# Xiaoming-Zhao/PointNav-VO

Hardware: AMD Instinct MI355X
Metric: RGB-D frame-pair VO inferences/s @341x192 (higher is better)
Workload: dtype f32

## Files before the change

include/pnvo.h:

```cpp
#ifndef PNVO_H_
#define PNVO_H_

#include <stddef.h>
#include <stdint.h>

#ifdef __cplusplus
extern "C" {
#endif

#define PNVO_OK 0
#define PNVO_ERR_ARG (-1)
#define PNVO_ERR_HIP (-2)
#define PNVO_ERR_STATE (-3)
#define PNVO_ERR_WEIGHTS (-4)
#define PNVO_ERR_INPUT (-5)

typedef struct pnvo_model_s *pnvo_handle;

typedef struct {
  int32_t width, height;
  int32_t n_rgb, n_depth, n_dd, n_tdv;
  int32_t baseplanes;
  int32_t hidden;
  int32_t out_dim;
// ... 129 lines not shown

int pnvo_policy_act(pnvo_policy_handle h, const float *depth, const float *goal, const int64_t *prev_actions,
                    const float *masks, const float *hidden_in, int B, float *hidden_out, float *features, float *logits,
                    float *value, void *stream);

int pnvo_policy_features_shape(pnvo_policy_handle h, int64_t shape[3]);
int pnvo_policy_encode(pnvo_policy_handle h, const float *depth, int B, float *features_out, void *stream);
int pnvo_policy_act_features(pnvo_policy_handle h, const float *visual_features, const float *goal, const int64_t *prev_actions,
                             const float *masks, const float *hidden_in, int B, float *hidden_out, float *features, float *logits,
                             float *value, void *stream);

int pnvo_policy_destroy(pnvo_policy_handle h);

size_t pnvo_policy_train_tail_floats(pnvo_policy_handle h);
int pnvo_policy_train_attach(pnvo_policy_handle h, float *params, float *grads, size_t n_floats, const pnvo_tensor_desc *toc,
                             int ntoc);

int pnvo_policy_train_refresh(pnvo_policy_handle h, void *stream);

int pnvo_policy_evaluate(pnvo_policy_handle h, const float *depth, const float *goal, const int64_t *prev_actions,
                         const float *masks, const float *hidden_in, int T, int N, const int64_t *actions, int train_encoder,
                         float *hidden_out, float *value, float *logp, float *entropy, void *stream);

int pnvo_policy_evaluate_features(pnvo_policy_handle h, const float *visual_features, const float *goal, const int64_t *prev_actions,
                                  const float *masks, const float *hidden_in, int T, int N, const int64_t *actions, float *hidden_out,
                                  float *value, float *logp, float *entropy, void *stream);

int pnvo_policy_ppo_loss(pnvo_policy_handle h, const float *actions_logp_old, const float *adv, const float *value_preds,
                         const float *returns, float clip, float value_coef, float entropy_coef, int use_clipped_value_loss,
                         float *out3, void *stream);

int pnvo_policy_backward(pnvo_policy_handle h, int train_encoder, void *stream);

int pnvo_policy_clip_grad_norm(pnvo_policy_handle h, float max_norm, float *norm_out, void *stream);

int pnvo_policy_train_timing(pnvo_policy_handle h, int mode);
int pnvo_policy_train_timing_read(pnvo_policy_handle h, double ms[5]);


int pnvo_rollout_insert(float *recurrent_hidden_states, int64_t *actions, int64_t *prev_actions, float *action_log_probs,
                        float *value_preds, float *rewards, float *masks, int T, int N, int64_t hidden_row, int step,
                        const float *hidden_in, const int64_t *actions_in, const float *action_log_probs_in,
                        const float *value_preds_in, const float *rewards_in, const float *masks_in, void *stream);

int pnvo_rollout_after_update(float *recurrent_hidden_states, int64_t *prev_actions, float *masks, int T, int N, int64_t hidden_row,
                              int step, void *stream);

int pnvo_rollout_compute_returns(const float *rewards, float *value_preds, const float *masks, float *returns, const float *next_value,
                                 int T, int N, int step, int use_gae, float gamma, float gamma_tau, void *stream);

int pnvo_rollout_gather(const float *recurrent_hidden_states, const int64_t *actions, const int64_t *prev_actions,
                        const float *value_preds, const float *returns, const float *masks, const float *action_log_probs,
                        const float *advantages, const int64_t *perm, int N, int L, int H, int steps, int start, int n_mb,
                        float *hidden_out, int64_t *actions_out, int64_t *prev_actions_out, float *value_preds_out, float *returns_out,
                        float *masks_out, float *action_log_probs_out, float *advantages_out, void *stream);

int pnvo_rollout_gather_frames(const float *frames, const int64_t *perm, int N, int64_t F, int steps, int start, int n_mb, float *out,
                               void *stream);

int pnvo_avgpool2(const float *depth, int N, int H, int W, float *out, void *stream);

const char *pnvo_last_error(pnvo_handle h);

const char *pnvo_last_note(pnvo_handle h);


int pnvo_set_tap(pnvo_handle h, const char *name, float *dst, size_t capacity);
int pnvo_tap_shape(pnvo_handle h, const char *name, int B, int64_t shape[4]);

typedef struct {
  char name[96];
  int64_t launches;
  double total_ms;
  double flops;
  double bytes;
} pnvo_kernel_time;
int pnvo_forward_features(pnvo_handle h, const float *rgb, const float *depth, const float *dd, const float *tdv,
                          const int64_t *actions, int B, float *hidden_out, void *stream);

int pnvo_check_inputs(pnvo_handle h);

int pnvo_layer_kernel(pnvo_handle h, const char *name, int B, char *family, size_t cap, double *executed_flops);

int pnvo_timing_mode(pnvo_handle h, int mode);
int pnvo_timing_read(pnvo_handle h, pnvo_kernel_time *entries, int cap, int *n_out);

size_t pnvo_packed_conv_floats(int cout, int cin, int kh, int kw);
int pnvo_pack_conv_weight(const float *oihw, int cout, int cin, int kh, int kw, float *out);

int pnvo_resize_area(const void *src, int src_dtype, int n, int in_h, int in_w, int channels, int64_t src_frame_stride,
                     int64_t src_row_stride, int64_t src_pix_stride, int rs_h, int rs_w, int crop_y, int crop_x, int out_h, int out_w,
                     float *dst, int dst_group, int64_t dst_group_stride, int64_t dst_member_stride, int64_t dst_row_stride,
                     int64_t dst_pix_stride, int div_rule, void *stream);

const char *pnvo_version(void);

long long pnvo_device_bytes_live(void);

#ifdef __cplusplus
}
#endif
#endif
```

pointnav-vo_amd/_lib.py:

```python
import ctypes as C
import os

import numpy as np

import torch

_HERE = os.path.dirname(os.path.abspath(__file__))
LIB_PATH = os.path.join(_HERE, "csrc", "libpnvo.so")

PNVO_OK = 0


GRAD_READY_FN = C.CFUNCTYPE(None, C.c_void_p, C.c_uint64, C.c_uint64, C.c_void_p)


class PnvoError(RuntimeError):
    pass


class pnvo_config(C.Structure):
    _fields_ = [(n, C.c_int32) for n in (
        "width", "height", "n_rgb", "n_depth", "n_dd", "n_tdv", "baseplanes", "hidden", "out_dim", "normalize",
        "act_embed", "n_acts", "flat_size", "max_batch", "backbone_depth")]

# ... 18 lines not shown
                                        C.c_void_p, C.c_void_p]),
    "pnvo_forward_grouped_raw": (C.c_int, [C.c_void_p, C.c_void_p, C.c_int, C.c_void_p, C.c_void_p, C.c_void_p, C.c_int, C.c_void_p,
                                           C.c_void_p, C.c_void_p]),
    "pnvo_grouped_supported": (C.c_int, [C.c_void_p, C.c_int]),
    "pnvo_set_precision": (C.c_int, [C.c_void_p, C.c_int]),
    "pnvo_set_option": (C.c_int, [C.c_void_p, C.c_char_p, C.c_char_p]),
    "pnvo_get_option": (C.c_int, [C.c_void_p, C.c_char_p, C.c_char_p, C.c_size_t]),
    "pnvo_forward_dual": (C.c_int, [C.c_void_p, C.c_void_p, C.c_void_p, C.c_void_p, C.c_void_p, C.c_void_p, C.c_int,
                                    C.c_void_p, C.c_void_p, C.c_void_p]),
    "pnvo_build_obs_pairs": (C.c_int, [C.c_void_p, C.c_void_p, C.c_int, C.c_int, C.c_int, C.c_int, C.POINTER(C.c_float), C.c_int,
                                       C.c_void_p, C.c_void_p, C.c_void_p, C.c_void_p, C.c_void_p, C.c_void_p, C.c_void_p]),
    "pnvo_stage_frames": (C.c_int, [C.c_void_p, C.c_int, C.c_size_t, C.c_void_p, C.c_int]),
    "pnvo_stage_frames2": (C.c_int, [C.c_void_p, C.c_size_t, C.c_void_p, C.c_void_p, C.c_size_t, C.c_void_p, C.c_int, C.c_int]),
    "pnvo_discretize_depth": (C.c_int, [C.c_void_p, C.c_int64, C.c_int64, C.c_int, C.c_void_p, C.c_int64, C.c_void_p,
                                        C.c_void_p]),
    "pnvo_topdown_workspace_bytes": (C.c_size_t, [C.c_int, C.c_int, C.c_int]),
    "pnvo_topdown_view_f64": (C.c_int, [C.c_void_p, C.c_int, C.c_int, C.c_int, C.c_int64, C.c_int64, C.c_void_p, C.c_int,
                                        C.c_void_p, C.c_int64, C.c_int64, C.c_void_p, C.c_void_p]),
    "pnvo_half_to_float": (C.c_int, [C.c_void_p, C.c_int64, C.c_void_p, C.c_void_p]),
    "pnvo_dataset_pairs": (C.c_int, [C.c_void_p] * 7 + [C.c_int] * 5 + [C.c_void_p] * 7),
    "pnvo_topdown_view_pairs": (C.c_int, [C.c_void_p, C.c_int, C.c_int, C.c_int, C.POINTER(C.c_float), C.c_int, C.c_void_p, C.c_void_p,
                                          C.c_void_p]),
    "pnvo_topdown_view": (C.c_int, [C.c_void_p, C.c_int, C.c_int, C.c_int, C.c_int64, C.c_int64,
                                    C.POINTER(C.c_float), C.c_int, C.c_void_p, C.c_int64, C.c_int64, C.c_void_p,
                                    C.c_void_p]),
    "pnvo_train_attach": (C.c_int, [C.c_void_p, C.c_void_p, C.c_void_p, C.c_size_t, C.POINTER(pnvo_tensor_desc), C.c_int]),
    "pnvo_train_refresh": (C.c_int, [C.c_void_p, C.c_void_p]),
    "pnvo_train_forward": (C.c_int, [C.c_void_p, C.c_void_p, C.c_void_p, C.c_void_p, C.c_void_p, C.c_int, C.c_void_p,
                                     C.c_void_p, C.c_void_p, C.c_void_p]),
    "pnvo_train_backward": (C.c_int, [C.c_void_p, C.c_void_p, C.c_void_p]),
    "pnvo_train_set_grad_hook": (C.c_int, [C.c_void_p, C.c_void_p, C.c_void_p]),
    "pnvo_train_grad_buckets": (C.c_int, [C.c_void_p, C.POINTER(C.c_uint64), C.POINTER(C.c_uint64), C.c_int, C.POINTER(C.c_int)]),
    "pnvo_input_moments": (C.c_int, [C.c_void_p, C.c_void_p, C.c_void_p, C.c_void_p, C.c_void_p, C.c_int, C.c_void_p,
                                     C.c_int, C.c_void_p, C.c_void_p]),
    "pnvo_rmv_merge": (C.c_int, [C.c_void_p, C.c_int, C.c_int, C.c_void_p, C.c_void_p, C.c_void_p, C.c_void_p]),
    "pnvo_train_set_actions": (C.c_int, [C.c_void_p, C.c_void_p]),
    "pnvo_mse_loss": (C.c_int, [C.c_void_p, C.c_void_p, C.c_int, C.c_int, C.c_void_p, C.c_void_p, C.c_void_p]),
    "pnvo_mse_loss_coef": (C.c_int, [C.c_void_p, C.c_void_p, C.c_void_p, C.c_int, C.c_void_p, C.c_void_p, C.c_void_p]),
    "pnvo_geo_inverse_loss": (C.c_int, [C.c_void_p, C.c_void_p, C.c_int, C.c_int, C.c_float, C.c_void_p, C.c_void_p,
                                        C.c_void_p]),
    "pnvo_train_set_dropout": (C.c_int, [C.c_void_p, C.c_float, C.c_uint64]),
    "pnvo_train_dropout_mask": (C.c_int, [C.c_void_p, C.c_int, C.c_void_p, C.c_void_p]),
    "pnvo_adam_step": (C.c_int, [C.c_void_p, C.c_void_p, C.c_void_p, C.c_void_p, C.c_size_t, C.c_float, C.c_float,
                                 C.c_float, C.c_float, C.c_int, C.c_void_p]),
    "pnvo_destroy": (C.c_int, [C.c_void_p]),
    "pnvo_ring_assemble": (C.c_int, [C.c_void_p, C.c_void_p, C.c_void_p, C.c_void_p, C.c_void_p, C.c_void_p, C.c_void_p, C.c_int, C.c_int,
                                     C.c_int, C.c_void_p, C.c_void_p, C.c_void_p, C.c_void_p]),
    "pnvo_last_error": (C.c_char_p, [C.c_void_p]),
    "pnvo_last_note": (C.c_char_p, [C.c_void_p]),
    "pnvo_set_tap": (C.c_int, [C.c_void_p, C.c_char_p, C.c_void_p, C.c_size_t]),
    "pnvo_tap_shape": (C.c_int, [C.c_void_p, C.c_char_p, C.c_int, C.POINTER(C.c_int64)]),
    "pnvo_check_inputs": (C.c_int, [C.c_void_p]),
    "pnvo_forward_features": (C.c_int, [C.c_void_p, C.c_void_p, C.c_void_p, C.c_void_p, C.c_void_p, C.c_void_p, C.c_int,
                                        C.c_void_p, C.c_void_p]),
    "pnvo_policy_create": (C.c_int, [C.c_void_p, C.c_int, C.POINTER(C.c_void_p)]),
    "pnvo_policy_load_weights": (C.c_int, [C.c_void_p, C.c_void_p, C.c_size_t, C.c_void_p, C.c_int]),
    "pnvo_policy_act": (C.c_int, [C.c_void_p, C.c_void_p, C.c_void_p, C.c_void_p, C.c_void_p, C.c_void_p, C.c_int,
                                  C.c_void_p, C.c_void_p, C.c_void_p, C.c_void_p, C.c_void_p]),
    "pnvo_policy_features_shape": (C.c_int, [C.c_void_p, C.POINTER(C.c_int64)]),
    "pnvo_policy_encode": (C.c_int, [C.c_void_p, C.c_void_p, C.c_int, C.c_void_p, C.c_void_p]),
    "pnvo_policy_act_features": (C.c_int, [C.c_void_p, C.c_void_p, C.c_void_p, C.c_void_p, C.c_void_p, C.c_void_p, C.c_int,
                                           C.c_void_p, C.c_void_p, C.c_void_p, C.c_void_p, C.c_void_p]),
    "pnvo_policy_evaluate_features": (C.c_int, [C.c_void_p, C.c_void_p, C.c_void_p, C.c_void_p, C.c_void_p, C.c_void_p, C.c_int, C.c_int,
                                                C.c_void_p, C.c_void_p, C.c_void_p, C.c_void_p, C.c_void_p, C.c_void_p]),
    "pnvo_policy_destroy": (C.c_int, [C.c_void_p]),
    "pnvo_policy_train_tail_floats": (C.c_size_t, [C.c_void_p]),
    "pnvo_policy_train_attach": (C.c_int, [C.c_void_p, C.c_void_p, C.c_void_p, C.c_size_t, C.POINTER(pnvo_tensor_desc), C.c_int]),
    "pnvo_policy_train_refresh": (C.c_int, [C.c_void_p, C.c_void_p]),
    "pnvo_policy_evaluate": (C.c_int, [C.c_void_p, C.c_void_p, C.c_void_p, C.c_void_p, C.c_void_p, C.c_void_p, C.c_int, C.c_int,
                                       C.c_void_p, C.c_int, C.c_void_p, C.c_void_p, C.c_void_p, C.c_void_p, C.c_void_p]),
    "pnvo_policy_ppo_loss": (C.c_int, [C.c_void_p, C.c_void_p, C.c_void_p, C.c_void_p, C.c_void_p, C.c_float, C.c_float, C.c_float,
                                       C.c_int, C.c_void_p, C.c_void_p]),
    "pnvo_policy_backward": (C.c_int, [C.c_void_p, C.c_int, C.c_void_p]),
    "pnvo_policy_clip_grad_norm": (C.c_int, [C.c_void_p, C.c_float, C.c_void_p, C.c_void_p]),
    "pnvo_policy_train_timing": (C.c_int, [C.c_void_p, C.c_int]),
    "pnvo_policy_train_timing_read": (C.c_int, [C.c_void_p, C.POINTER(C.c_double)]),
    "pnvo_rollout_insert": (C.c_int, [C.c_void_p] * 7 + [C.c_int, C.c_int, C.c_int64, C.c_int] + [C.c_void_p] * 7),
    "pnvo_rollout_after_update": (C.c_int, [C.c_void_p] * 3 + [C.c_int, C.c_int, C.c_int64, C.c_int, C.c_void_p]),
    "pnvo_rollout_compute_returns": (C.c_int, [C.c_void_p] * 5 + [C.c_int] * 4 + [C.c_float, C.c_float, C.c_void_p]),
    "pnvo_rollout_gather": (C.c_int, [C.c_void_p] * 9 + [C.c_int] * 6 + [C.c_void_p] * 9),
    "pnvo_rollout_gather_frames": (C.c_int, [C.c_void_p, C.c_void_p, C.c_int, C.c_int64] + [C.c_int] * 3 + [C.c_void_p, C.c_void_p]),
    "pnvo_avgpool2": (C.c_int, [C.c_void_p, C.c_int, C.c_int, C.c_int, C.c_void_p, C.c_void_p]),
    "pnvo_layer_kernel": (C.c_int, [C.c_void_p, C.c_char_p, C.c_int, C.c_char_p, C.c_size_t, C.POINTER(C.c_double)]),
    "pnvo_timing_mode": (C.c_int, [C.c_void_p, C.c_int]),
    "pnvo_timing_read": (C.c_int, [C.c_void_p, C.POINTER(pnvo_kernel_time), C.c_int, C.POINTER(C.c_int)]),
    "pnvo_packed_conv_floats": (C.c_size_t, [C.c_int, C.c_int, C.c_int, C.c_int]),
    "pnvo_pack_conv_weight": (C.c_int, [C.c_void_p, C.c_int, C.c_int, C.c_int, C.c_int, C.c_void_p]),
    "pnvo_resize_area": (C.c_int, [C.c_void_p, C.c_int, C.c_int, C.c_int, C.c_int, C.c_int, C.c_int64, C.c_int64, C.c_int64,
                                   C.c_int, C.c_int, C.c_int, C.c_int, C.c_int, C.c_int, C.c_void_p, C.c_int, C.c_int64, C.c_int64,
                                   C.c_int64, C.c_int64, C.c_int, C.c_void_p]),
    "pnvo_version": (C.c_char_p, []),
    "pnvo_device_bytes_live": (C.c_longlong, []),
}


def _load():
    if not os.path.exists(LIB_PATH):
        raise PnvoError(
            f"{LIB_PATH} is missing: the HIP extension has not been built.  Run "
            "`python -c 'import __graft_entry__ as g; g.build()'` (or `make -C pointnav-vo_amd/csrc`).  "
            "There is no CPU fallback.")
    lib = C.CDLL(LIB_PATH)
    for name, (res, args) in _SIGNATURES.items():
        fn = getattr(lib, name)
        fn.restype = res
        fn.argtypes = args
    return lib


lib = _load()


def check(rc, handle=None):
    if rc != PNVO_OK:
        msg = lib.pnvo_last_error(handle)
        raise PnvoError(f"libpnvo error {rc}: {msg.decode() if msg else '?'}")


def make_toc(entries):
    toc = (pnvo_tensor_desc * len(entries))()
    for i, (name, offset, shape) in enumerate(entries):
        toc[i].name = name.encode()
        toc[i].offset = int(offset)
        toc[i].ndim = len(shape)
        for k, s in enumerate(shape):
            toc[i].shape[k] = int(s)
    return toc


def pack_tensors(named_tensors):
    blob = np.ascontiguousarray(np.concatenate(
        [t.detach().to("cpu", torch.float32).reshape(-1).numpy() for _, t in named_tensors]), dtype=np.float32)
    entries, off = [], 0
    for name, t in named_tensors:
        entries.append((name, off, tuple(t.shape)))
        off += t.numel()
    return blob, make_toc(entries)


def version():
    return lib.pnvo_version().decode()
```

pointnav-vo_amd/csrc/conv_rows.hip:

```cpp
#include <cstdio>
#include <cstdlib>

#include "pnvo_internal.h"

namespace pnvo {

typedef float f32x16 __attribute__((ext_vector_type(16)));
typedef float f32x4 __attribute__((ext_vector_type(4)));
typedef float f32x2 __attribute__((ext_vector_type(2)));
typedef _Float16 f16x8 __attribute__((ext_vector_type(8)));
typedef _Float16 f16x2 __attribute__((ext_vector_type(2)));
typedef unsigned u32x4 __attribute__((ext_vector_type(4)));
typedef unsigned u32x2 __attribute__((ext_vector_type(2)));

#ifndef PNVO_ROWS_ABL
#define PNVO_ROWS_ABL 0
#endif
#if PNVO_ROWS_ABL
#define RS_DBG(p) ((p).rs_dbg)
#else
#define RS_DBG(p) 0
#endif

namespace {
constexpr int RS_THREADS = 512;
constexpr int RS_HG = 128;
constexpr int RS_RING = 512;
constexpr int RS_TAIL = 48;
constexpr int RS_PITCH = 144;
constexpr int RS_RAW = (RS_RING + RS_TAIL) * RS_PITCH;
constexpr int RS_OTAB = RS_RAW + 4 * 16384;
constexpr int RS_MTAB = RS_OTAB + 4 * RS_HG * 4;
constexpr int RS_SS = RS_MTAB + 4 * RS_HG * 4;
constexpr int RS_RED = RS_SS + 64 * 4;
constexpr int RS_DOF = RS_RED + 8 * 32 * 2 * 4;
constexpr int RS_LDS = RS_DOF + 512 * 16;

__device__ __forceinline__ void rs_barrier() { asm volatile("s_waitcnt lgkmcnt(0)\n\ts_barrier" ::: "memory"); }

__device__ __forceinline__ unsigned rs_pack2h(float a, float b) {
  const f16x2 r = __builtin_convertvector(f32x2{a, b}, f16x2);
  return __builtin_bit_cast(unsigned, r);
}
}

template <int MODE>
__global__ __launch_bounds__(RS_THREADS) __attribute__((amdgpu_waves_per_eu(2, 2))) void conv_rows32_kernel(const ConvX3Args p) {
  extern __shared__ __attribute__((aligned(16))) unsigned char lds[];
  const int tid = (int)threadIdx.x;
  const int lane = tid & 63;
  const int wave = __builtin_amdgcn_readfirstlane(tid >> 6);
  const int set = wave >> 2, sw = wave & 3, stid = tid & 255;
  const int H = p.H, W = p.W, P = W + 2;
  const int nbands = p.rs_bands, brows = p.rs_rows;
  const int nitems = p.B * nbands;
  const int dR = (2 * RS_HG) / P, dC = 2 * RS_HG - dR * P;

  u32x4 bres[18][2];
#pragma unroll
  for (int st = 0; st < 18; ++st)
#pragma unroll
    for (int pc = 0; pc < 2; ++pc)
      bres[st][pc] = *reinterpret_cast<const u32x4 *>(reinterpret_cast<const char *>(p.wpk) + (size_t)st * 2048u + pc * 1024 + lane * 16);
  const float os = p.oscale_ptr != nullptr ? *p.oscale_ptr : p.oscale;

  const int q = stid & 7, jb = stid >> 3;
  int q_ = q, jb_ = jb, lane_ = lane;
  unsigned *otab = reinterpret_cast<unsigned *>(lds + RS_OTAB) + set * 2 * RS_HG;
  float *mtab = reinterpret_cast<float *>(lds + RS_MTAB) + set * 2 * RS_HG;
  float *red = reinterpret_cast<float *>(lds + RS_RED);
  float *sstab = reinterpret_cast<float *>(lds + RS_SS);
  const unsigned rawbase = (unsigned)(RS_RAW + set * 32768 + sw * 4096);

  const unsigned tbytes = (unsigned)p.B * (unsigned)(H * W * 128);
  const __amdgpu_buffer_rsrc_t rx = __builtin_amdgcn_make_buffer_rsrc((void *)p.x, 0, tbytes, 0x00020000);
  const __amdgpu_buffer_rsrc_t ry = __builtin_amdgcn_make_buffer_rsrc((void *)p.y, 0, tbytes, 0x00020000);
  const __amdgpu_buffer_rsrc_t rres = __builtin_amdgcn_make_buffer_rsrc((void *)(MODE == 2 ? p.res : p.x), 0, tbytes, 0x00020000);
  const __amdgpu_buffer_rsrc_t rxo = __builtin_amdgcn_make_buffer_rsrc((void *)(MODE >= 2 ? p.xout : p.y), 0, tbytes, 0x00020000);

  for (int item = (int)blockIdx.x; item < nitems; item += (int)gridDim.x) {
    const int n = item / nbands, band = item - n * nbands;
    const int rb = band * brows, re = min(H, rb + brows);
    const int O0 = (rb + 1) * P;
    const int nout = (re - rb) * P;
    const int NH = (nout + RS_HG - 1) / RS_HG;
    const int nbase = n * H * W * 128;
    if (MODE >= 1 && tid < 64) sstab[tid] = tid < 32 ? p.in_scale[(size_t)n * 32 + tid] : p.in_shift[(size_t)n * 32 + tid - 32];
    const int r_lo = max(rb - 1, 0), r_hi = min(re, H - 1);
    int iR, iC, iD;
    {
      const int f = O0 - 2 * RS_HG + RS_HG * (1 + set) + jb + 256 * P;
      iR = f / P - 256;
      iC = f - (iR + 256) * P;
      iD = (((iR - 1) * W + iC - 1) * 32 + 4 * q) * 4 + nbase;
    }
    int oR = 0, oC = 0, oD = 0;
    if (stid < RS_HG) {
      const int f = O0 + RS_HG * set + stid;
      oR = f / P;
      oC = f - oR * P;
      oD = ((oR - 1) * W + oC - 1) * 128 + nbase;
    }

    unsigned vok = 0, vokn = 0;
    u32x4 *const dofp = reinterpret_cast<u32x4 *>(lds + RS_DOF) + tid;
    auto issue = [&](int slot) {
      vokn = 0;
      unsigned off[4];
      u32x4 dn = {0, 0, 0, 0};
#pragma unroll
      for (int k = 0; k < 4; ++k) {
        const int r32 = (32 * k) / P, c32 = 32 * k - r32 * P;
        const int cw = iC + c32 >= P ? 1 : 0;
        const int R = iR + r32 + cw, Cc = iC + c32 - cw * P;
        const bool ok = (unsigned)(R - 1 - r_lo) <= (unsigned)(r_hi - r_lo) && (unsigned)(Cc - 1) < (unsigned)W;
        const unsigned dense = (unsigned)(iD + (32 * k - 2 * (r32 + cw)) * 128), absent = ok ? 0u : 0x80000000u;
        off[k] = ok ? dense - 1024u * k : 0x80000000u;
        vokn |= ok ? (1u << k) : 0u;
        if (MODE >= 2) {
          dn[k] = dense | absent;
          vokn |= (ok && (unsigned)(R - 1 - rb) < (unsigned)(re - rb)) ? (16u << k) : 0u;
        }
      }
      if (MODE >= 2) *dofp = dn;
      if (!(RS_DBG(p) & 1)) {
        const unsigned m0v = rawbase + (unsigned)slot * 16384u;
        asm volatile(
            "s_mov_b32 m0, %5\n\ts_nop 0\n\t"
            "buffer_load_dwordx4 %0, %4, 0 offen lds\n\t"
            "buffer_load_dwordx4 %1, %4, 0 offen offset:1024 lds\n\t"
// ... 120 lines not shown
          a[1] = *reinterpret_cast<const u32x4 *>(lds + arow[0] + 64);
#pragma unroll
          for (int st = 0; st < 18; ++st) {
            if (st + 1 < 18) {
              const int nt = (st + 1) >> 1, nk = (st + 1) & 1;
              an[0] = *reinterpret_cast<const u32x4 *>(lds + arow[nt / 3] + (nt % 3) * RS_PITCH + nk * 32);
              an[1] = *reinterpret_cast<const u32x4 *>(lds + arow[nt / 3] + (nt % 3) * RS_PITCH + nk * 32 + 64);
            }
            f32x16 &c = (TWO_ACC && (st & 1)) ? acc1 : acc;
            c = __builtin_amdgcn_mfma_f32_32x32x16_f16(__builtin_bit_cast(f16x8, a[1]), __builtin_bit_cast(f16x8, bres[st][0]), c, 0, 0, 0);
            c = __builtin_amdgcn_mfma_f32_32x32x16_f16(__builtin_bit_cast(f16x8, a[0]), __builtin_bit_cast(f16x8, bres[st][1]), c, 0, 0, 0);
            c = __builtin_amdgcn_mfma_f32_32x32x16_f16(__builtin_bit_cast(f16x8, a[0]), __builtin_bit_cast(f16x8, bres[st][0]), c, 0, 0, 0);
            a[0] = an[0];
            a[1] = an[1];
          }
          if (TWO_ACC) {
#pragma unroll
            for (int r = 0; r < 16; ++r) acc[r] += acc1[r];
          }
          if (EPI_IN_COMPUTE) epilogue(h);
        }
      } else {
        asm volatile("s_waitcnt vmcnt(0)" ::: "memory");
#if PNVO_ROWS_ABL
        pt1 = __builtin_readcyclecounter();
        pc_wait += pt1 - pt0;
#endif
        asm volatile("" : "+v"(q_), "+v"(jb_), "+v"(lane_));
        vok = vokn;
        if (MODE >= 2) dof = *dofp;
        if (MODE == 2) load_skip();
        if (h + 6 <= NH + 2) issue((duty + 1) & 1);
        if (!EPI_IN_COMPUTE && h >= 1) epilogue(h - 1);
        if (h + 4 <= NH + 2 && !(RS_DBG(p) & 8)) convert_store(h + 4, duty & 1);

        if (h + 1 >= 0 && h + 1 < NH) tables(h + 1);
        ++duty;
      }
#if PNVO_ROWS_ABL
      const unsigned long long pt2 = __builtin_readcyclecounter();
      if ((h & 1) == set) pc_compute += pt2 - pt0; else pc_stage += pt2 - pt1;
#endif
      rs_barrier();
#if PNVO_ROWS_ABL
      pc_bar += __builtin_readcyclecounter() - pt2;
#endif
    }
#if PNVO_ROWS_ABL
    if (p.prof != nullptr && item == 7 && lane == 0) {
      unsigned long long *d = p.prof + wave * 8;
      d[0] = pc_compute; d[1] = pc_stage; d[2] = pc_bar; d[3] = pc_wait; d[4] = (unsigned long long)(NH + 4);
    }
#endif

    if (p.stats != nullptr) {
      t1 += __shfl_xor(t1, 32);
      t2 += __shfl_xor(t2, 32);
      if (lane < 32) *reinterpret_cast<f32x2 *>(red + (wave * 32 + lane) * 2) = f32x2{t1, t2};
      __syncthreads();
      if (wave == 0 && lane < 32) {
        float s1 = 0.f, s2 = 0.f;
#pragma unroll
        for (int w = 0; w < 8; ++w) {
          const f32x2 o = *reinterpret_cast<const f32x2 *>(red + (w * 32 + lane) * 2);
          s1 += o[0];
          s2 += o[1];
        }
        float *dst = p.stats + (((size_t)n * p.slots + band) * 32 + lane) * 2;
        dst[0] = s1;
        dst[1] = s2;
        if (p.gn_scale != nullptr) {
          const int c = lane;
          const bool first = p.gn_mu != nullptr && c % p.gn_cpg == 0;
          const long gi = (long)n * (32 / p.gn_cpg) + c / p.gn_cpg;
          gn_finalize_lane(s1, s2, p.gn_cpg, p.gn_P, p.gn_eps, p.gn_gamma[c], p.gn_beta[c], p.gn_scale + (size_t)n * 32 + c,
                           p.gn_shift + (size_t)n * 32 + c, first ? p.gn_mu + gi : nullptr, first ? p.gn_rstd + gi : nullptr);
        }
      }
    }
    __syncthreads();
  }
}

bool conv_rows32_plan(ConvX3Args &a, int ks, int stride, int mode, int num_cus) {
  if (ks != 3 || stride != 1 || a.np != 2 || a.CIN != 32 || a.COUTP != 32 || a.in_absmax != nullptr) return false;
  if (mode < 0 || mode > 3 || (mode == 2 && a.res_scale != nullptr)) return false;
  if (a.Ho != a.H || a.Wo != a.W || a.W + 3 > RS_HG || a.W < 8 || a.H < 8 || (long)a.B * a.H * a.W * 128 >= (1L << 31)) return false;
  int bands = 1;
  while ((long)a.B * bands < num_cus && bands < 4 && a.H / (bands * 2) >= 12) bands *= 2;
  if ((long)a.B * bands < num_cus) return false;
  if (const char *e = std::getenv("PNVO_ROWS_DBG")) a.rs_dbg = std::atoi(e);
  a.rs_rows = (a.H + bands - 1) / bands;
  a.rs_bands = (a.H + a.rs_rows - 1) / a.rs_rows;
  a.slots = a.rs_bands;
  return true;
}

hipError_t launch_conv_rows32(const ConvX3Args &a, int mode, int num_cus, hipStream_t s) {
  static std::mutex attr_mu;
  static unsigned long long attr_seen = 0;
  if (pnvo_first_launch_on_device(attr_mu, attr_seen)) {
    hipError_t e = hipFuncSetAttribute(reinterpret_cast<const void *>(conv_rows32_kernel<0>), hipFuncAttributeMaxDynamicSharedMemorySize, RS_LDS);
    if (e == hipSuccess)
      e = hipFuncSetAttribute(reinterpret_cast<const void *>(conv_rows32_kernel<1>), hipFuncAttributeMaxDynamicSharedMemorySize, RS_LDS);
    if (e == hipSuccess)
      e = hipFuncSetAttribute(reinterpret_cast<const void *>(conv_rows32_kernel<2>), hipFuncAttributeMaxDynamicSharedMemorySize, RS_LDS);
    if (e == hipSuccess)
      e = hipFuncSetAttribute(reinterpret_cast<const void *>(conv_rows32_kernel<3>), hipFuncAttributeMaxDynamicSharedMemorySize, RS_LDS);
    if (e != hipSuccess) return e;
  }
  const long items = (long)a.B * a.rs_bands;
  const unsigned gx = (unsigned)(items < num_cus ? items : num_cus);
  ConvX3Args q = a;
#if PNVO_ROWS_ABL
  static unsigned long long *prof = nullptr;
  if (std::getenv("PNVO_ROWS_PROF") != nullptr) {
    if (!prof && hipMalloc((void **)&prof, 8 * 8 * 8) != hipSuccess) return hipErrorOutOfMemory;
    (void)hipMemsetAsync(prof, 0, 8 * 8 * 8, s);
    q.prof = prof;
  }
#endif
  if (mode == 0)
    hipLaunchKernelGGL((conv_rows32_kernel<0>), dim3(gx), dim3(RS_THREADS), RS_LDS, s, q);
  else if (mode == 1)
    hipLaunchKernelGGL((conv_rows32_kernel<1>), dim3(gx), dim3(RS_THREADS), RS_LDS, s, q);
  else if (mode == 2)
    hipLaunchKernelGGL((conv_rows32_kernel<2>), dim3(gx), dim3(RS_THREADS), RS_LDS, s, q);
  else if (mode == 3)
    hipLaunchKernelGGL((conv_rows32_kernel<3>), dim3(gx), dim3(RS_THREADS), RS_LDS, s, q);
  else
    return hipErrorInvalidValue;
#if PNVO_ROWS_ABL
  if (q.prof != nullptr) {
    unsigned long long h[64];
    (void)hipStreamSynchronize(s);
    (void)hipMemcpy(h, prof, sizeof(h), hipMemcpyDeviceToHost);
    for (int w = 0; w < 8; w += 3)
      std::fprintf(stderr, "[pnvo] conv_rows32 wave %d: per half-step (cycles): compute role %.0f  stage role %.0f (+ wait for its loads/stores %.0f)  barrier %.0f  (%llu half-steps)\n",
                   w, 2.0 * h[8 * w] / h[8 * w + 4], 2.0 * h[8 * w + 1] / h[8 * w + 4], 2.0 * h[8 * w + 3] / h[8 * w + 4], (double)h[8 * w + 2] / h[8 * w + 4], h[8 * w + 4]);
  }
#endif
  return hipGetLastError();
}

}
```

pointnav-vo_amd/csrc/conv_x3.hip:

```cpp
#include <cmath>
#include <cstdio>
#include <cstdlib>
#include <cstring>

#include "pnvo_internal.h"

namespace pnvo {

typedef float f32x16 __attribute__((ext_vector_type(16)));
typedef float f32x4 __attribute__((ext_vector_type(4)));
typedef float f32x2 __attribute__((ext_vector_type(2)));
typedef __bf16 bf16x8 __attribute__((ext_vector_type(8)));
typedef __bf16 bf16x2 __attribute__((ext_vector_type(2)));
typedef _Float16 f16x8 __attribute__((ext_vector_type(8)));
typedef _Float16 f16x2 __attribute__((ext_vector_type(2)));
typedef unsigned u32x4 __attribute__((ext_vector_type(4)));

namespace {
__device__ __forceinline__ unsigned pack2(float a, float b) {
  const bf16x2 r = __builtin_convertvector(f32x2{a, b}, bf16x2);
  return __builtin_bit_cast(unsigned, r);
}
__device__ __forceinline__ unsigned pack2h(float a, float b) {
  const f16x2 r = __builtin_convertvector(f32x2{a, b}, f16x2);
  return __builtin_bit_cast(unsigned, r);
}
__device__ __forceinline__ float lo_f(unsigned u) { return __builtin_bit_cast(float, u << 16); }
__device__ __forceinline__ float hi_f(unsigned u) { return __builtin_bit_cast(float, u & 0xffff0000u); }
}

constexpr int x3_wpe(int mw, int nw, int np, bool dsf = false) {
  return dsf ? (mw * nw >= 6 ? 1 : (mw * nw >= 2 ? 2 : 3)) : ((np == 2 && mw * nw <= 2) ? 3 : 2);
}

template <int KS, int STRIDE, int MODE, int MW, int NW, int NP, bool DSF = false, bool W8 = false, bool KSW = false>
__global__ __launch_bounds__(W8 ? 512 : 256) __attribute__((amdgpu_waves_per_eu(W8 ? 2 : x3_wpe(MW, NW, NP, DSF), W8 ? 2 : x3_wpe(MW, NW, NP, DSF)))) void conv_x3_kernel(const ConvX3Args p) {
  constexpr int NTH = W8 ? 512 : 256, NWV = NTH / 64;
  constexpr int EMW = KSW ? 1 : MW;
  static_assert(!KSW || (NW == 1 && NP == 2 && KS == 3 && !DSF && !W8), "K split over the waves: float16-piece 3x3 convs, one N-tile");
  static_assert(!DSF || (KS == 3 && STRIDE == 2 && NP == 2 && (MODE == 0 || MODE == 2)), "the downsample rides on a float16-piece 3x3 stride-2 conv");
  extern __shared__ __attribute__((aligned(16))) unsigned char lds[];
  constexpr int PSTEP = KS == 1 ? STRIDE : 1;
  constexpr int CS = KS == 1 ? 1 : STRIDE;
  constexpr int PAD = KS / 2;
  const int lane = threadIdx.x & 63;
  const int wave = __builtin_amdgcn_readfirstlane(threadIdx.x >> 6);

  const int ntiles = p.B * p.tiles_r * p.tiles_c;
  const int chunk = (ntiles + 7) >> 3;
  int bid = (int)(blockIdx.x & 7) * chunk + (int)(blockIdx.x >> 3);
  if (bid >= ntiles) return;
  const int tci = bid % p.tiles_c;
  bid /= p.tiles_c;
  const int tri = bid % p.tiles_r;
  const int n = bid / p.tiles_r;
  const int r0 = tri * p.TR, c0 = tci * p.TC;
  const int hi0 = r0 * STRIDE - PAD, wi0 = c0 * STRIDE - PAD;
  const int mdl = (p.grp_end0 > 0 && n >= p.grp_end0) + (p.grp_end1 > 0 && n >= p.grp_end1);
  const unsigned short *g_wpk = mdl == 0 ? p.wpk : p.wpk_g[mdl - 1];
  const unsigned short *g_ds_wpk = mdl == 0 ? p.ds_wpk : p.ds_wpk_g[mdl - 1];
  const float g_oscale = mdl == 0 ? p.oscale : p.oscale_g[mdl - 1], g_ds_oscale = mdl == 0 ? p.ds_oscale : p.ds_oscale_g[mdl - 1];
  const float *g_gamma = mdl == 0 ? p.gn_gamma : p.gn_gamma_g[mdl - 1], *g_beta = mdl == 0 ? p.gn_beta : p.gn_beta_g[mdl - 1];
  const float *g_ds_gamma = mdl == 0 ? p.ds_gamma : p.ds_gamma_g[mdl - 1], *g_ds_beta = mdl == 0 ? p.ds_beta : p.ds_beta_g[mdl - 1];
  const int PR = p.PR, PC = p.PC, CK = p.CK;
  const int pitch = CK * 2 + 16;
  const int plane = PR * PC * pitch;
  const int npix = p.TR * p.TC;
  const int tab_off = KSW ? max(NP * plane, 4 * MW * 4096) : NP * plane;
  unsigned *qtab = reinterpret_cast<unsigned *>(lds + tab_off);
  unsigned *otab = qtab + p.MT * 32;
  for (int e = (int)threadIdx.x; e < p.MT * 32; e += NTH) {
    const int q = min(e, npix - 1);
    const int tr = q / p.TC, tc = q - tr * p.TC;
    qtab[e] = (unsigned)(((tr * CS) * PC + tc * CS) * pitch);
    const bool ok = e < npix && r0 + tr < p.Ho && c0 + tc < p.Wo;
    otab[e] = (unsigned)((tr * p.Wo + tc) * p.COUTP) | (ok ? 0u : 0x80000000u);
  }

  const int wn = p.wn;
  const int wave_m = wave / wn;
  const int wave_n = (wave & (wn - 1)) + (int)blockIdx.y * wn;
  const int ntt = p.COUTP >> 5, kct = p.CIN >> 4;

  f32x16 acc[MW][NW];
#pragma unroll
  for (int i = 0; i < MW; ++i)
#pragma unroll
    for (int j = 0; j < NW; ++j)
#pragma unroll
      for (int r = 0; r < 16; ++r) acc[i][j][r] = 0.f;
  f32x16 accd[DSF ? MW : 1][DSF ? NW : 1];
  if (DSF) {
#pragma unroll
    for (int i = 0; i < MW; ++i)
#pragma unroll
      for (int j = 0; j < NW; ++j)
#pragma unroll
        for (int r = 0; r < 16; ++r) accd[DSF ? i : 0][DSF ? j : 0][r] = 0.f;
  }

  float in_mul = 1.f, in_div = 1.f;
  const bool in_scaled = NP == 2 && p.in_absmax != nullptr;
  if (in_scaled) {
    unsigned mb = p.in_absmax[(threadIdx.x & 63) * 16];
#pragma unroll
    for (int d = 32; d >= 1; d >>= 1) mb = max(mb, (unsigned)__shfl_xor((int)mb, d));
    const int e = mb != 0u ? (int)((mb >> 23) & 0xffu) - 126 : 14;
    in_mul = __builtin_bit_cast(float, (unsigned)(14 - e + 127) << 23);
    in_div = __builtin_bit_cast(float, (unsigned)(e - 14 + 127) << 23);
  }
  const int G = CK >> 3;
  const int cg = threadIdx.x & (G - 1), pl = threadIdx.x / G, PS = NTH / G;
  const int dr = PS / PC, dc = PS - dr * PC;
  const int nppix = PR * PC;

  unsigned long long c_stage = 0, c_mm = 0, t_0 = __builtin_readcyclecounter(), r_0 = wall_clock64();
  for (int ck0 = 0; ck0 < p.CIN; ck0 += CK) {
    unsigned long long t_a = __builtin_readcyclecounter();
    if (ck0 > 0) __syncthreads();
// ... 416 lines not shown
      u32x4 ent[4];
#pragma unroll
      for (int g4 = 0; g4 < 4; ++g4) ent[g4] = *reinterpret_cast<const u32x4 *>(otab + mt * 32 + 8 * g4 + 4 * rr16);
      unsigned flags = 0;
#pragma unroll
      for (int g4 = 0; g4 < 4; ++g4) flags |= ent[g4][0] | ent[g4][1] | ent[g4][2] | ent[g4][3];
      const bool whole = !__any((int)(flags >> 31));
#pragma unroll
      for (int j = 0; j < NW; ++j) {
        const int nt = wave_n * NW + j;
        if (nt >= ntt) continue;
        const int co = nt * 32 + (lane & 31);
        float s1 = 0.f, s2 = 0.f;
        if (whole) {
#pragma unroll
          for (int r = 0; r < 16; ++r) {
            const float v = ac[i][j][r];
            (yout + ybase + co)[ent[r >> 2][r & 3]] = v;
            s1 += v;
            s2 = __builtin_fmaf(v, v, s2);
          }
        } else {
#pragma unroll
          for (int r = 0; r < 16; ++r) {
            const unsigned e = ent[r >> 2][r & 3];
            const bool ok = (int)e >= 0;
            const float v = ok ? ac[i][j][r] : 0.f;
            if (ok) (yout + ybase + co)[e] = v;
            s1 += v;
            s2 = __builtin_fmaf(v, v, s2);
          }
        }
        t1[j] += s1 + __shfl_xor(s1, 32);
        t2[j] += s2 + __shfl_xor(s2, 32);
      }
    }
    if (stats != nullptr) {
      const int rows = NWV / wn;
      float *red = reinterpret_cast<float *>(lds);
      if (rows > 1) {
        __syncthreads();
        if (lane < 32)
#pragma unroll
          for (int j = 0; j < NW; ++j) *reinterpret_cast<f32x2 *>(red + ((wave * NW + j) * 32 + lane) * 2) = f32x2{t1[j], t2[j]};
        __syncthreads();
      }
      if (wave_m == 0 && lane < 32) {
#pragma unroll
        for (int j = 0; j < NW; ++j) {
          const int nt = wave_n * NW + j;
          if (nt >= ntt) continue;
          float s1 = t1[j], s2 = t2[j];
          for (int w = 1; w < rows; ++w) {
            const f32x2 o = *reinterpret_cast<const f32x2 *>(red + (((w * wn + (wave & (wn - 1))) * NW + j) * 32 + lane) * 2);
            s1 += o[0];
            s2 += o[1];
          }
          float *dst = stats + (((long)n * p.slots + tri * p.tiles_c + tci) * p.COUTP + nt * 32 + lane) * 2;
          dst[0] = s1;
          dst[1] = s2;
          if (gscale != nullptr) {
            const int c = nt * 32 + lane;
            const bool first = gmu != nullptr && c % p.gn_cpg == 0;
            const long gi = (long)n * (p.COUTP / p.gn_cpg) + c / p.gn_cpg;
            gn_finalize_lane(s1, s2, p.gn_cpg, p.gn_P, p.gn_eps, gamma[c], beta[c], gscale + (long)n * p.COUTP + c,
                             gshift + (long)n * p.COUTP + c, first ? gmu + gi : nullptr, first ? grstd + gi : nullptr);
          }
        }
      }
    }
    (void)again;
  };
  emit(acc, p.y, p.stats, p.oscale_ptr, g_oscale, g_gamma, g_beta, p.gn_scale, p.gn_shift, p.gn_mu, p.gn_rstd, false);
  if constexpr (DSF) emit(accd, p.ds_y, p.ds_stats, p.ds_oscale_ptr, g_ds_oscale, g_ds_gamma, g_ds_beta, p.ds_scale, p.ds_shift, p.ds_mu, p.ds_rstd, true);
  if (p.prof && lane == 0 && blockIdx.x == 13 && blockIdx.y == 0) {
    const unsigned long long t_f = __builtin_readcyclecounter();
    unsigned long long *d = p.prof + wave * 8;
    d[0] = c_stage;
    d[1] = c_mm;
    d[2] = t_f - t_e;
    d[3] = t_f - t_0;
    d[4] = wall_clock64() - r_0;
  }
}


template <int MODE, int MW, int NW, bool BRES>
__global__ __launch_bounds__(256) __attribute__((amdgpu_waves_per_eu(BRES ? 2 : 3, BRES ? 2 : 3))) void conv_x3p_kernel(const ConvX3Args p) {
  static_assert(MODE == 0 || MODE == 1 || MODE == 3, "the block-tail stager has no registers for a second patch");
  static_assert(!BRES || NW == 1, "resident weights: one N-tile");
  extern __shared__ __attribute__((aligned(16))) unsigned char lds[];
  constexpr int KS = 3, PAD = 1, NP = 2;
  const int lane = threadIdx.x & 63;
  const int wave = __builtin_amdgcn_readfirstlane(threadIdx.x >> 6);
  const int ntiles = p.B * p.tiles_r * p.tiles_c;
  const int chunk = (ntiles + 7) >> 3;
  const int PR = p.PR, PC = p.PC, CK = p.CK;
  const int pitch = CK * 2 + 16;
  const int plane = PR * PC * pitch;
  const int npix = p.TR * p.TC;
  unsigned *qtab = reinterpret_cast<unsigned *>(lds + NP * plane);
  unsigned *otab = qtab + p.MT * 32;
  const int wn = p.wn;
  const int wave_m = wave / wn;
  const int wave_n = (wave & (wn - 1)) + (int)blockIdx.y * wn;
  const int ntt = p.COUTP >> 5;
  float in_mul = 1.f, in_div = 1.f;
  const bool in_scaled = p.in_absmax != nullptr;
  if (in_scaled) {
    unsigned mb = p.in_absmax[(threadIdx.x & 63) * 16];
#pragma unroll
    for (int d = 32; d >= 1; d >>= 1) mb = max(mb, (unsigned)__shfl_xor((int)mb, d));
    const int e = mb != 0u ? (int)((mb >> 23) & 0xffu) - 126 : 14;
    in_mul = __builtin_bit_cast(float, (unsigned)(14 - e + 127) << 23);
    in_div = __builtin_bit_cast(float, (unsigned)(e - 14 + 127) << 23);
  }
  const int G = CK >> 3;
  const int cg = threadIdx.x & (G - 1), pl = threadIdx.x / G, PS = 256 / G;
  const int nppix = PR * PC;
  constexpr int NPX = 6;
  int ppr[NPX], ppc[NPX];
  unsigned poff[NPX];
  bool pok[NPX];
#pragma unroll
  for (int k = 0; k < NPX; ++k) {
    const int pix = pl + k * PS;
    pok[k] = pix < nppix;
    const int q = pok[k] ? pix : 0;
    ppr[k] = q / PC;
    ppc[k] = q - ppr[k] * PC;
    poff[k] = (unsigned)((ppr[k] * PC + ppc[k]) * pitch + 16 * cg);
  }
  if ((int)threadIdx.x < p.MT * 32) {
    const int q = min((int)threadIdx.x, npix - 1);
    const int tr = q / p.TC, tc = q - tr * p.TC;
    qtab[threadIdx.x] = (unsigned)((tr * PC + tc) * pitch);
  }
  struct Tile {
    int n, tri, tci, r0, c0, hi0, wi0;
    bool valid;
  };
  auto decode = [&](int vb) {
    Tile t;
    int bid = (vb & 7) * chunk + (vb >> 3);
    t.valid = vb < 8 * chunk && bid < ntiles;
    if (!t.valid) bid = 0;
    t.tci = bid % p.tiles_c;
    bid /= p.tiles_c;
    t.tri = bid % p.tiles_r;
    t.n = bid / p.tiles_r;
    t.r0 = t.tri * p.TR;
    t.c0 = t.tci * p.TC;
    t.hi0 = t.r0 - PAD;
    t.wi0 = t.c0 - PAD;
    return t;
  };
  f32x4 v[NPX][2], sc0, sc1, sh0, sh1;
  bool inb[NPX];
  auto fetch = [&](const Tile &t) {
    const long img = ((long)t.n * p.H * p.W) * p.CIN + 8 * cg;
    if (MODE >= 1) {
      const float *ps = p.in_scale + (long)t.n * p.CIN + 8 * cg;
      const float *pt = p.in_shift + (long)t.n * p.CIN + 8 * cg;
      sc0 = *reinterpret_cast<const f32x4 *>(ps);
      sc1 = *reinterpret_cast<const f32x4 *>(ps + 4);
      sh0 = *reinterpret_cast<const f32x4 *>(pt);
// ... 223 lines not shown
          }
        } else {
#pragma unroll
          for (int r = 0; r < 16; ++r) {
            const unsigned e = ent[r >> 2][r & 3];
            const bool ok = (int)e >= 0;
            const float x = ok ? acc[i][j][r] : 0.f;
            if (ok) (p.y + ybase + co)[e] = x;
            s1 += x;
            s2 = __builtin_fmaf(x, x, s2);
          }
        }
        t1[j] += s1 + __shfl_xor(s1, 32);
        t2[j] += s2 + __shfl_xor(s2, 32);
      }
    }
    if (p.stats != nullptr) {
      const int rows = 4 / wn;
      float *red = reinterpret_cast<float *>(lds);
      if (rows > 1) {
        __syncthreads();
        if (lane < 32)
#pragma unroll
          for (int j = 0; j < NW; ++j) *reinterpret_cast<f32x2 *>(red + ((wave * NW + j) * 32 + lane) * 2) = f32x2{t1[j], t2[j]};
        __syncthreads();
      }
      if (wave_m == 0 && lane < 32) {
#pragma unroll
        for (int j = 0; j < NW; ++j) {
          const int nt = wave_n * NW + j;
          if (nt >= ntt) continue;
          float s1 = t1[j], s2 = t2[j];
          for (int w = 1; w < rows; ++w) {
            const f32x2 o = *reinterpret_cast<const f32x2 *>(red + (((w * wn + (wave & (wn - 1))) * NW + j) * 32 + lane) * 2);
            s1 += o[0];
            s2 += o[1];
          }
          float *dst = p.stats + (((long)cur.n * p.slots + cur.tri * p.tiles_c + cur.tci) * p.COUTP + nt * 32 + lane) * 2;
          dst[0] = s1;
          dst[1] = s2;
        }
      }
    }
    if (!nxt.valid) break;
    if (BRES) fetch(nxt);
    __syncthreads();
    cur = nxt;
  }
}

namespace {
template <int KS, int STRIDE, int NP>
hipError_t launch_ks(const ConvX3Args &a, int mode, int mw, int nw, dim3 grid, size_t ldsb, hipStream_t s) {
#define PNVO_X3(MODE_, MW_, NW_)                                                                          \
  if (mode == MODE_ && mw == MW_ && nw == NW_) {                                                          \
    hipLaunchKernelGGL((conv_x3_kernel<KS, STRIDE, MODE_, MW_, NW_, NP>), grid, dim3(256), ldsb, s, a);   \
    return hipGetLastError();                                                                             \
  }
  if constexpr (KS == 3 && STRIDE == 2 && NP == 2) {
    if (a.ds_wpk != nullptr) {
#define PNVO_X3D(MODE_, MW_, NW_)                                                                               \
  if (mode == MODE_ && mw == MW_ && nw == NW_) {                                                                \
    hipLaunchKernelGGL((conv_x3_kernel<KS, STRIDE, MODE_, MW_, NW_, NP, true>), grid, dim3(256), ldsb, s, a);   \
    return hipGetLastError();                                                                                   \
  }
      if (a.w8) {
#define PNVO_X3DW(MODE_)                                                                                                  \
  if (mode == MODE_ && mw == 3 && nw == 1) {                                                                             \
    hipLaunchKernelGGL((conv_x3_kernel<KS, STRIDE, MODE_, 3, 1, NP, true, true>), grid, dim3(512), ldsb, s, a);          \
    return hipGetLastError();                                                                                            \
  }
        PNVO_X3DW(0) PNVO_X3DW(2)
#undef PNVO_X3DW
        return hipErrorInvalidValue;
      }
      PNVO_X3D(0, 1, 1) PNVO_X3D(2, 1, 1) PNVO_X3D(0, 2, 1) PNVO_X3D(2, 2, 1) PNVO_X3D(0, 2, 2) PNVO_X3D(2, 2, 2) PNVO_X3D(0, 3, 2) PNVO_X3D(2, 3, 2)
#undef PNVO_X3D
      return hipErrorInvalidValue;
    }
  }
  PNVO_X3(0, 1, 1) PNVO_X3(1, 1, 1) PNVO_X3(0, 2, 1) PNVO_X3(1, 2, 1) PNVO_X3(0, 2, 2) PNVO_X3(1, 2, 2) PNVO_X3(0, 3, 2) PNVO_X3(1, 3, 2)
  PNVO_X3(2, 1, 1) PNVO_X3(2, 2, 1) PNVO_X3(2, 2, 2) PNVO_X3(2, 3, 2) PNVO_X3(3, 1, 1) PNVO_X3(3, 2, 1) PNVO_X3(3, 2, 2) PNVO_X3(3, 3, 2)

  if (KS == 3 && STRIDE == 1 && NP == 2) {
    PNVO_X3(0, 5, 1) PNVO_X3(1, 5, 1) PNVO_X3(2, 5, 1) PNVO_X3(3, 5, 1)
    if constexpr (KS == 3 && STRIDE == 1 && NP == 2) if (a.ksw) {
#define PNVO_X3K(MODE_, MW_)                                                                                             \
  if (mode == MODE_ && mw == MW_ && nw == 1) {                                                                          \
    hipLaunchKernelGGL((conv_x3_kernel<KS, STRIDE, MODE_, MW_, 1, NP, false, false, true>), grid, dim3(256), ldsb, s, a); \
    return hipGetLastError();                                                                                           \
  }
      PNVO_X3K(0, 3) PNVO_X3K(1, 3) PNVO_X3K(2, 3) PNVO_X3K(0, 4) PNVO_X3K(1, 4) PNVO_X3K(2, 4)
#undef PNVO_X3K
      return hipErrorInvalidValue;
    }
  }
  if constexpr (KS == 3 && NP == 2) if (a.w8) {
#define PNVO_X3W(MODE_)                                                                                                  \
  if (mode == MODE_ && mw == 3 && nw == 1) {                                                                            \
  hipLaunchKernelGGL((conv_x3_kernel<KS, STRIDE, MODE_, 3, 1, NP, false, true>), grid, dim3(512), ldsb, s, a);        \
  return hipGetLastError();                                                                                           \
  }
    PNVO_X3W(0) PNVO_X3W(1) PNVO_X3W(2) PNVO_X3W(3)
#undef PNVO_X3W
    return hipErrorInvalidValue;
  }
#undef PNVO_X3
  return hipErrorInvalidValue;
}
}

namespace {
bool conv_x3_plan_impl(ConvX3Args &a, int ks, int stride, int *mw, int *nw, size_t *lds_bytes, bool fine);
long plan_wgs(const ConvX3Args &a, int nw) {
  const int ntt = a.COUTP / 32;
  return (long)a.B * a.tiles_r * a.tiles_c * ((ntt + a.wn * nw - 1) / (a.wn * nw));
}
}

bool conv_x3_plan(ConvX3Args &a, int ks, int stride, int *mw, int *nw, size_t *lds_bytes) {
  ConvX3Args reg = a;
  int rmw = 0, rnw = 0;
  size_t rlds = 0;
  const int force0 = a.force;
  reg.force = 1;
  const bool reg_ok = conv_x3_plan_impl(reg, ks, stride, &rmw, &rnw, &rlds, false);
  const long reg_wgs = reg_ok ? plan_wgs(reg, rnw) : 0;
  const int ntt = a.COUTP / 32;
  if (a.fine && a.np == 2 && ntt >= 2 && (!reg_ok || reg_wgs < 224)) {
    ConvX3Args f = a;
    int fmw = 0, fnw = 0;
    size_t flds = 0;
    f.force = 1;
    if (conv_x3_plan_impl(f, ks, stride, &fmw, &fnw, &flds, true)) {
      const long fw = plan_wgs(f, fnw);
      if (fw > reg_wgs && (fw >= 48 || force0)) {
        f.force = force0;
        a = f;
        *mw = fmw;
        *nw = fnw;
        *lds_bytes = flds;
        return true;
      }
    }
  }
  return conv_x3_plan_impl(a, ks, stride, mw, nw, lds_bytes, false);
}

namespace {
bool conv_x3_plan_impl(ConvX3Args &a, int ks, int stride, int *mw, int *nw, size_t *lds_bytes, bool fine) {
  if (a.CIN % 32 || a.COUTP % 32 || a.COUTP > 1024 || a.CIN > 1024) return false;
  if (!((ks == 3 && (stride == 1 || stride == 2)) || (ks == 1 && stride == 2))) return false;
  a.w8 = 0;
  a.ksw = 0;
  const int ntt = a.COUTP / 32;
  int TR, TC;
  if (stride == 2 && ks == 3) {
    TC = a.Wo >= 32 ? 16 : a.Wo;
    const int pc = 2 * TC + 1;
    TR = (324 / pc - 1) / 2;
    if (TR < 1) return false;
    if (TR > a.Ho) TR = a.Ho;
    while (TR > 1 && TR * TC > (ntt == 2 ? 64 : (ntt == 4 ? 128 : 96))) --TR;
  } else if (ntt == 1 && stride == 1 && ks == 3 && a.CIN > 32 && a.np == 2 && a.Wo < 32 && a.Ho * a.Wo <= 128) {
    TC = a.Wo;
    TR = a.Ho;
  } else if (ntt == 1) {
    if (stride != 1 || ks != 3 || a.CIN != 32) return false;
    TC = a.Wo >= 16 ? 16 : a.Wo;
    TR = 256 / TC;
    while (TR > 1 && (TR + 2) * (TC + 2) > 324) --TR;
    if (TR > a.Ho) TR = a.Ho;
    if (TR * TC <= 96) return false;
  } else if (a.strip && !fine && a.np == 2 && stride == 1 && ks == 3 && ntt == 4 && a.Wo >= 16 && a.Ho >= 8) {
    const int ncol = (a.Wo + 21) / 22;
    TC = (a.Wo + ncol - 1) / ncol;
    TR = 288 / TC;
    if (TR > a.Ho) TR = a.Ho;
    const int nrow = (a.Ho + TR - 1) / TR;
    TR = (a.Ho + nrow - 1) / nrow;
  } else if (a.Wo >= 32) {
    TR = 8;
    TC = 16;
  } else {
    TC = a.Wo;
    int target = ntt == 4 ? 192 : (ntt >= 8 ? 96 : 128);
    if (fine && a.ksw_ok && ks == 3 && stride == 1 && a.np == 2 && a.CIN >= 128) target = 96;
    TR = target / TC;
    if (TR < 1) TR = 1;
    if (TR > a.Ho) TR = a.Ho;
  }
  a.TR = TR;
  a.TC = TC;
  a.tiles_r = (a.Ho + TR - 1) / TR;
  a.tiles_c = (a.Wo + TC - 1) / TC;
  a.MT = (TR * TC + 31) / 32;
  const int cs = ks == 1 ? 1 : stride;
  a.PR = (TR - 1) * cs + ks;
  a.PC = (TC - 1) * cs + ks;
  const bool strip = a.strip && !fine && a.np == 2 && stride == 1 && ks == 3 && ntt == 4 && a.Wo >= 16 && a.Ho >= 8 && a.MT > 6;
  if (fine) {
    if (a.MT > 8) return false;
    a.wn = 1;
    *mw = (a.MT + 3) / 4;
    *nw = 1;
    if (a.ksw_ok && (a.MT == 3 || a.MT == 4) && ks == 3 && stride == 1 && a.np == 2 && a.CIN >= 128) {
      a.ksw = 1;
      *mw = a.MT;
    }
  } else if (strip) {
    a.wn = 2;
    *mw = (a.MT + 1) / 2;
    *nw = 1;
    if (*mw > 5) return false;
    if (*mw < 5) *mw = 5;
  } else if (ntt == 1) {
    a.wn = 1;
    *mw = a.CIN > 32 ? 1 : 2;
    *nw = 1;
    if (a.ksw_ok && a.CIN >= 128 && (a.MT == 3 || a.MT == 4) && ks == 3 && stride == 1 && a.np == 2) {
      a.ksw = 1;
      *mw = a.MT;
    }
  } else if (ntt == 2) {
    a.wn = 2;
    *mw = a.MT > 2 ? 2 : 1;
    *nw = 1;
  } else if (ntt == 4) {
    a.wn = 2;
    *mw = a.MT > 4 ? 3 : 2;
    *nw = 2;
  } else {
    a.wn = 4;
    *mw = a.MT > 2 ? 3 : 2;
    *nw = 2;
    const long ntiles = (long)a.B * a.tiles_r * a.tiles_c;
    if (ntiles < 200 && a.MT <= 4) {
      a.wn = 2;
      *mw = 2;
    }
    if (a.w8_ok && !fine && ntiles >= 200 && a.MT == 3 && ntt == 8 && a.np == 2 && ks == 3) {
      a.w8 = 1;
      a.wn = 8;
      *mw = 3;
      *nw = 1;
    }
  }
  if (!a.ksw && ((a.w8 ? 8 : 4) / a.wn) * *mw < a.MT) return false;
  const size_t np = a.np == 2 ? 2 : 3;
  int ck = 32;
  while (ck < 256 && a.CIN % (2 * ck) == 0) ck *= 2;
  const size_t cap = (size_t)72 * 1024;
  while (ck > 32 && np * a.PR * a.PC * (ck * 2 + 16) > cap) ck /= 2;
  if (np * a.PR * a.PC * (ck * 2 + 16) > cap + 4096) return false;
  if (a.CIN % ck) return false;
  a.CK = ck;
  {
    const bool force = a.force != 0;
    const long wgs = (long)a.B * a.tiles_r * a.tiles_c * ((ntt + a.wn * *nw - 1) / (a.wn * *nw));
    if (wgs < (a.np == 2 ? 112 : 192) && !force) return false;
  }
  a.slots = a.tiles_r * a.tiles_c;
  *lds_bytes = np * a.PR * a.PC * (ck * 2 + 16) + (size_t)a.MT * 32 * 4 * 2;
  if (a.ksw) *lds_bytes = std::max(np * a.PR * a.PC * (ck * 2 + 16), (size_t)4 * a.MT * 4096) + (size_t)a.MT * 32 * 4 * 2;
  return true;
}
}

bool conv_x3_persistent(const ConvX3Args &a, int ks, int stride, int mode, int mw, int nw) {
  const long ntiles = (long)a.B * a.tiles_r * a.tiles_c;
  const int ntt = a.COUTP / 32, pwgs = a.persist_wgs;
  const bool bres = ntt == 1 && a.CIN == 32 && nw == 1 && (mode == 0 || mode == 1);
  return a.np == 2 && ks == 3 && stride == 1 && bres && mw * nw <= 2 && a.CK == a.CIN && pwgs >= 8 &&
         (long)a.PR * a.PC * (a.CK / 8) <= 6 * 256 && ntiles >= 2L * pwgs;
}

hipError_t launch_conv_x3(const ConvX3Args &a0, int ks, int stride, int mode, int mw, int nw, size_t lds_bytes, hipStream_t s) {
  ConvX3Args a = a0;
  static unsigned long long *prof = nullptr;
  static const bool want = std::getenv("PNVO_X3_PROF") != nullptr;
  if (want && !prof) {
    (void)hipMalloc((void **)&prof, 512);
    (void)hipMemset(prof, 0, 512);
  }
  a.prof = prof;
  struct Dump {
    const ConvX3Args &a; int mw, nw; hipStream_t s; unsigned long long *prof;
    ~Dump() {
      static int calls = 0;
      if (!prof || ++calls > 40) return;
      unsigned long long h[64];
      (void)hipStreamSynchronize(s);
      (void)hipMemcpy(h, prof, 512, hipMemcpyDeviceToHost);
      std::fprintf(stderr, "[pnvo] conv_x3 B %d %dx%d cin %d cout %d tile %dx%d MT %d CK %d (%d,%d) wn %d: wave0 stage %llu mfma %llu epi %llu total %llu "
                           "(100MHz ticks %llu) | wave3 stage %llu mfma %llu epi %llu total %llu\n", a.B, a.Ho, a.Wo, a.CIN, a.COUTP, a.TR, a.TC,
                   a.MT, a.CK, mw, nw, a.wn, h[0], h[1], h[2], h[3], h[4], h[24], h[25], h[26], h[27]);
    }
  } dump{a, mw, nw, s, prof};
  const long ntiles = (long)a.B * a.tiles_r * a.tiles_c;
  const int ntt = a.COUTP / 32, per_wg = a.wn * nw;
  dim3 grid((unsigned)(((ntiles + 7) / 8) * 8), (unsigned)((ntt + per_wg - 1) / per_wg), 1u);
  const int pwgs = a.persist_wgs;
  if (conv_x3_persistent(a, ks, stride, mode, mw, nw)) {
    const bool bres = true;
    dim3 pg((unsigned)(pwgs & ~7), grid.y, 1u);
    if (bres) pg.x = (unsigned)(((pwgs / 3) * 2) & ~7);
#define PNVO_X3P(MODE_, MW_, NW_)                                                                        \
  if (mode == MODE_ && mw == MW_ && nw == NW_) {                                                         \
    hipLaunchKernelGGL((conv_x3p_kernel<MODE_, MW_, NW_, true>), pg, dim3(256), lds_bytes, s, a);       \
    return hipGetLastError();                                                                            \
  }
    PNVO_X3P(0, 1, 1) PNVO_X3P(1, 1, 1) PNVO_X3P(0, 2, 1) PNVO_X3P(1, 2, 1)
#undef PNVO_X3P
  }
  if (a.np == 2) {
    if (ks == 3 && stride == 1) return launch_ks<3, 1, 2>(a, mode, mw, nw, grid, lds_bytes, s);
    if (ks == 3 && stride == 2) return launch_ks<3, 2, 2>(a, mode, mw, nw, grid, lds_bytes, s);
    if (ks == 1 && stride == 2) return launch_ks<1, 2, 2>(a, mode, mw, nw, grid, lds_bytes, s);
    return hipErrorInvalidValue;
  }
  if (ks == 3 && stride == 1) return launch_ks<3, 1, 3>(a, mode, mw, nw, grid, lds_bytes, s);
  if (ks == 3 && stride == 2) return launch_ks<3, 2, 3>(a, mode, mw, nw, grid, lds_bytes, s);
  if (ks == 1 && stride == 2) return launch_ks<1, 2, 3>(a, mode, mw, nw, grid, lds_bytes, s);
  return hipErrorInvalidValue;
}

void pack_conv_x3_weight(const float *oihw, int cout, int cin, int cinp, int coutp, int kh_, int kw_, unsigned short *out) {
  const int T = kh_ * kw_, kct = cinp / 16, ntt = coutp / 32;
  auto bf = [](float f) {
    unsigned u;
    std::memcpy(&u, &f, 4);
    if ((u & 0x7f800000u) == 0x7f800000u) return (unsigned short)(u >> 16);
    u += 0x7fffu + ((u >> 16) & 1u);
    return (unsigned short)(u >> 16);
  };
  auto tof = [](unsigned short h) {
    const unsigned u = (unsigned)h << 16;
    float f;
    std::memcpy(&f, &u, 4);
    return f;
  };
  for (int tap = 0; tap < T; ++tap)
    for (int kc = 0; kc < kct; ++kc)
      for (int nt = 0; nt < ntt; ++nt)
        for (int ln = 0; ln < 64; ++ln)
          for (int j = 0; j < 8; ++j) {
            const int co = nt * 32 + (ln & 31), ci = 16 * kc + 8 * (ln >> 5) + j;
            float v = 0.f;
            if (co < cout && ci < cin) v = oihw[((size_t)co * cin + ci) * T + tap];
            const unsigned short h = bf(v);
            const float r1 = v - tof(h);
            const unsigned short m = bf(r1);
            const unsigned short l = bf(r1 - tof(m));
            const size_t base = ((((size_t)tap * kct + kc) * ntt + nt) * 3) * 64 * 8 + (size_t)ln * 8 + j;
            out[base] = h;
            out[base + 64 * 8] = m;
            out[base + 2 * 64 * 8] = l;
          }
}

static unsigned short f32_to_f16_rne(float f) {
  const _Float16 h = (_Float16)f;
  unsigned short u;
  std::memcpy(&u, &h, 2);
  return u;
}
static float f16_to_f32(unsigned short u) {
  _Float16 h;
  std::memcpy(&h, &u, 2);
  return (float)h;
}
float pack_conv_x2_weight(const float *oihw, int cout, int cin, int cinp, int coutp, int kh_, int kw_, unsigned short *out) {
  const int T = kh_ * kw_, kct = cinp / 16, ntt = coutp / 32;
  float mx = 0.f;
  for (size_t k = 0; k < (size_t)cout * cin * T; ++k) mx = std::fmax(mx, std::fabs(oihw[k]));
  int e = 0;
  if (mx > 0.f) std::frexp(mx, &e);
  const float scale = std::ldexp(1.0f, 12 - e), inv = std::ldexp(1.0f, e - 12);
  for (int tap = 0; tap < T; ++tap)
    for (int kc = 0; kc < kct; ++kc)
      for (int nt = 0; nt < ntt; ++nt)
        for (int ln = 0; ln < 64; ++ln)
          for (int j = 0; j < 8; ++j) {
            const int co = nt * 32 + (ln & 31), ci = 16 * kc + 8 * (ln >> 5) + j;
            float v = 0.f;
            if (co < cout && ci < cin) v = oihw[((size_t)co * cin + ci) * T + tap] * scale;
            const unsigned short h = f32_to_f16_rne(v);
            const unsigned short m = f32_to_f16_rne(v - f16_to_f32(h));
            const size_t base = ((((size_t)tap * kct + kc) * ntt + nt) * 2) * 64 * 8 + (size_t)ln * 8 + j;
            out[base] = h;
            out[base + 64 * 8] = m;
          }
  return inv;
}

__global__ __launch_bounds__(256) void conv_x3_repack_kernel(const float *w, int cout, int cin, int cinp, int coutp, int T,
                                                           int transposed, unsigned short *out, long total) {
  const long e = (long)blockIdx.x * 256 + threadIdx.x;
  if (e >= total) return;
  const int j = (int)(e & 7), ln = (int)((e >> 3) & 63);
  long r = e >> 9;
  const int ntt = coutp / 32, kct = cinp / 16;
  const int nt = (int)(r % ntt);
  r /= ntt;
  const int kc = (int)(r % kct), tap = (int)(r / kct);
  const int co = nt * 32 + (ln & 31), ci = 16 * kc + 8 * (ln >> 5) + j;
  const float v = (co < cout && ci < cin) ? (transposed ? w[((long)ci * cout + co) * T + (T - 1 - tap)] : w[((long)co * cin + ci) * T + tap])
// ... 86 lines not shown
```

pointnav-vo_amd/csrc/pnvo_api.hip:

```cpp
#include <hip/hip_runtime.h>

#include <cmath>
#include <cstdio>
#include <cstdlib>
#include <cstring>
#include <functional>
#include <atomic>
#include <condition_variable>
#include <map>
#include <mutex>
#include <string>
#include <thread>
#include <vector>

#include "pnvo_model.h"

using namespace pnvo;

thread_local std::string g_err;

int pnvo_fail(pnvo_handle h, int code, const std::string &msg) {
  if (h) h->err = msg;
  g_err = msg;
  return code;
}

long long pnvo_device_bytes_live(void) { return g_device_bytes_live.load(); }

namespace {

inline int fail(pnvo_handle h, int code, const std::string &msg) { return pnvo_fail(h, code, msg); }


Layer make_layer(const std::string &name, const std::string &gn, int cin, int cout, int k, int stride, int pad,
                 int hin, int win, int groups) {
  Layer l;
  l.name = name;
  l.gn = gn;
  l.cin = cin;
  l.cinp = rup(cin, 8);
  l.cout = cout;
  l.coutp = rup(cout, 32);
  l.k = l.kw = k;
  l.stride = stride;
  l.pad = pad;
  l.hin = hin;
  l.win = win;
  l.hout = (hin + 2 * pad - k) / stride + 1;
  l.wout = (win + 2 * pad - k) / stride + 1;
  l.groups = groups;
  return l;
}

void build_plan(pnvo_model_s *m) {
  const pnvo_config &c = m->cfg;
  m->C = c.n_rgb + c.n_depth + c.n_dd + c.n_tdv;
  m->CP = rup(m->C, 8);
  m->CPL = rup(m->C, 16);
  m->Hs = halve(c.height);
  m->Ws = halve(c.width);
  m->Hp = halve(m->Hs);
  m->Wp = halve(m->Ws);
  {
    const int n[4] = {c.n_rgb, c.n_depth, c.n_dd, c.n_tdv};
    int prev_off[4], half = 0;
    for (int t = 0; t < 4; ++t) {
      prev_off[t] = half;
      half += n[t] / 2;
    }
    m->stem_ref_of_new.clear();
    m->stem_tensor_of_new.clear();
    m->stem_ch_of_new.clear();
    for (int t = 0; t < 4; ++t)
      for (int ch = 0; ch < n[t]; ++ch) {
        const int hn = n[t] / 2;
        m->stem_ref_of_new.push_back(ch < hn ? prev_off[t] + ch : half + prev_off[t] + (ch - hn));
        m->stem_tensor_of_new.push_back(t);
        m->stem_ch_of_new.push_back(ch);
      }
    while ((int)m->stem_ref_of_new.size() < m->CP) {
      m->stem_ref_of_new.push_back(-1);
      m->stem_tensor_of_new.push_back(-1);
      m->stem_ch_of_new.push_back(0);
    }
  }
  const int g = c.baseplanes / 2;
  const std::string bb = "visual_encoder.backbone.";
  m->convs.clear();
  m->convs.push_back(make_layer(bb + "conv1.0", bb + "conv1.1", m->C, c.baseplanes, 7, 2, 3, c.height, c.width, g));
  int h = m->Hp, w = m->Wp, cin = c.baseplanes;
  const bool bott = c.backbone_depth == 50 || c.backbone_depth == 101;
  const int nblk[4] = {bott ? 3 : 2, bott ? 4 : 2, bott ? (c.backbone_depth == 101 ? 23 : 6) : 2, bott ? 3 : 2};
  m->bottleneck = bott;
  m->blocks.clear();
  auto push = [&](Layer l) {
    l.block = (int)m->blocks.size();
    m->convs.push_back(std::move(l));
// ... 74 lines not shown
    s += "])";
    *rc = fail(h, PNVO_ERR_WEIGHTS, s);
    return nullptr;
  }
  return t.blob + d->offset;
}

}

void pnvo_pack_conv_weight_cinp(const float *oihw, int cout, int cin, int cinp, int kh, int kw, std::vector<float> &out) {
  const int coutp = rup(cout, 32), J = cinp / 8, T = kh * kw, ntg_n = coutp / 32;
  out.assign((size_t)coutp * cinp * T, 0.f);
  for (int ntg = 0; ntg < ntg_n; ++ntg)
    for (int tap = 0; tap < T; ++tap)
      for (int j = 0; j < J; ++j)
        for (int hh = 0; hh < 2; ++hh)
          for (int n = 0; n < 32; ++n)
            for (int t = 0; t < 4; ++t) {
              const int co = ntg * 32 + n, ci = 8 * j + 4 * hh + t;
              if (co < cout && ci < cin)
                out[((((size_t)ntg * T + tap) * J + j) * 64 + hh * 32 + n) * 4 + t] =
                    oihw[((size_t)co * cin + ci) * T + tap];
            }
}

namespace {
inline void pack_conv_weight_cinp(const float *oihw, int cout, int cin, int cinp, int kh, int kw, std::vector<float> &out) {
  pnvo_pack_conv_weight_cinp(oihw, cout, cin, cinp, kh, kw, out);
}

int load_conv(pnvo_handle h, const Toc &t, Layer &l, bool has_gn) {
  int rc = PNVO_OK;
  const float *w = find_tensor(h, t, l.name + ".weight", {l.cout, l.cin, l.k, l.kw}, &rc);
  if (!w) return rc;
  std::vector<float> pk;
  pack_conv_weight_cinp(w, l.cout, l.cin, l.cinp, l.k, l.kw, pk);
  HIPCHK(h, l.wpk.upload(pk.data(), pk.size()));
  l.host_w.assign(w, w + (size_t)l.cout * l.cin * l.k * l.kw);
  if (has_gn) {
    const float *g = find_tensor(h, t, l.gn + ".weight", {l.cout}, &rc);
    if (!g) return rc;
    const float *b = find_tensor(h, t, l.gn + ".bias", {l.cout}, &rc);
    if (!b) return rc;
    HIPCHK(h, l.gamma.upload(g, l.cout));
    HIPCHK(h, l.beta.upload(b, l.cout));
  }
  return PNVO_OK;
}

int reset_contract_flag(pnvo_handle h) {
  if (!h->dd_flag) HIPCHK(h, h->dd_flag.alloc_host(1, hipHostMallocMapped | hipHostMallocCoherent));
  if (!h->dd_flag_dev) HIPCHK(h, h->dd_flag_dev.alloc(1));
  *(volatile int *)h->dd_flag = 0;
  HIPCHK(h, hipMemset(h->dd_flag_dev, 0, sizeof(int)));
  return PNVO_OK;
}

void free_workspace(pnvo_model_s *m) {
  pnvo_drop_graphs(m);
  for (DevBuf<float> *b : {&m->xin, &m->stem_raw, &m->out_ws, &m->bufY[0], &m->bufY[1], &m->rawA, &m->rawB, &m->rawD, &m->rawC, &m->comp_raw,
                           &m->hid, &m->stats, &m->stats_ds, &m->tapbuf})
    b->reset();
  for (DevPair<float> *q : {&m->ssA, &m->ssB, &m->ssD, &m->ssC}) q->reset();
  m->cap = 0;
}

bool x3_layer(pnvo_handle m, const Layer &l) {
  const bool s2 = l.stride == 2 && m->opt.x3_s2;
  const bool k3 = l.k == 3 && l.kw == 3 && l.pad == 1 && (l.stride == 1 || s2);
  const bool k1 = l.k == 1 && l.kw == 1 && l.pad == 0 && s2;
  return (k3 || k1) && !l.host_w.empty() && m->opt.conv <= 1;
}
bool x3_two_pieces(pnvo_handle m, const Layer &l) {
  if (m->bottleneck || !(l.in_bound < 6.0e4f)) return false;
  if (m->train != nullptr)
    return m->opt.train_pieces == 2 && pnvo_train_x2_scale(m, l.name + ".weight") != nullptr;
  return m->opt.pieces == 2;
}
void x3_fill(pnvo_handle m, const Layer &l, int B, ConvX3Args &xa) {
  std::memset(&xa, 0, sizeof(xa));
  xa.force = m->opt.conv == 1;
  xa.strip = m->opt.x3_strip;
  xa.fine = m->opt.x3_fine;
  xa.w8_ok = m->opt.x3_w8;
  xa.ksw_ok = m->opt.x3_ksplit;
  xa.persist_wgs = m->opt.x3_persist ? 3 * m->num_cus : 0;
  xa.np = x3_two_pieces(m, l) ? 2 : 3;
  xa.B = B;
  xa.H = l.hin;
  xa.W = l.win;
  xa.CIN = l.cinp;
  xa.Ho = l.hout;
  xa.Wo = l.wout;
  xa.COUTP = l.coutp;
}
bool x3_args(pnvo_handle m, const Layer &l, int B, ConvX3Args &xa, int *mw, int *nw, size_t *ldsb) {
  x3_fill(m, l, B, xa);
  return conv_x3_plan(xa, l.k, l.stride, mw, nw, ldsb);
}

void conv_geometry(const Layer &l, int B, int y_cstride, ConvArgs &a) {
  std::memset(&a, 0, sizeof(a));
  a.B = B;
  a.H = l.hin;
  a.W = l.win;
  a.CIN = l.cinp;
  a.Ho = l.hout;
  a.Wo = l.wout;
  a.COUT = l.cout;
  a.COUTP = l.coutp;
  a.KH = l.k;
  a.KW = l.kw;
  a.stride = l.stride;
  a.pad = l.pad;
  a.y_cstride = y_cstride;
  a.up = 1;
}

bool layer_on_lds(pnvo_handle m, const Layer &l, int *slots) {
  ConvArgs a;
  conv_geometry(l, 0, l.coutp, a);
  if (!conv3_lds_supported(a) || m->opt.conv == 3) return false;
  if (slots) *slots = conv3_lds_slots(a);
  return true;
}

size_t stats_floats(pnvo_handle m, const Layer &l, int B) {
  const long P = (long)l.hout * l.wout, M = (long)B * P;
  int MT, NT;
  choose_tile(M, l.coutp, &MT, &NT);
  int slots = conv_slots((int)P, MT), s2 = 0;
  if (layer_on_lds(m, l, &s2) && s2 > slots) slots = s2;
  if ((l.k == 3 && l.kw == 3 && l.pad == 1 && (l.stride == 1 || l.stride == 2)) || (l.k == 1 && l.stride == 2)) {
    ConvX3Args xa;
    x3_fill(m, l, B, xa);
    xa.force = 1;
    int mw, nw;
    size_t ldsb;
    if (conv_x3_plan(xa, l.k, l.stride, &mw, &nw, &ldsb) && xa.slots > slots) slots = xa.slots;
  }
  return (size_t)B * (size_t)slots * l.coutp * 2;
}

int stem_slots(pnvo_handle m, StemPlan::Kernel k) {
  if (k == StemPlan::GENERIC) return 0;
  if (k == StemPlan::LDS) return stem_tiles_x(m->Ws) * stem_tiles_y(m->Hs);
  return k == StemPlan::MX ? stem_mx_slots(m->Hs, m->Ws) : stem_dd_slots(m->Hs, m->Ws);
}

int ensure_workspace(pnvo_handle m, int B) {
  if (B <= m->cap) return PNVO_OK;
  free_workspace(m);
  const pnvo_config &c = m->cfg;
  const size_t npix = (size_t)B * c.height * c.width;
  size_t act = (size_t)B * m->Hp * m->Wp * c.baseplanes;
  for (size_t k = 1; k < m->convs.size(); ++k) {
    const size_t need = (size_t)B * m->convs[k].hout * m->convs[k].wout * m->convs[k].coutp;
    if (need > act) act = need;
  }
  int maxc = m->comp_cp;
  size_t st = 0;
  for (StemPlan::Kernel k : {StemPlan::MX, StemPlan::DD, StemPlan::LDS}) st = std::max(st, (size_t)B * stem_slots(m, k) * m->convs[0].coutp * 2);
  for (const Layer &l : m->convs) {
    if (l.coutp > maxc) maxc = l.coutp;
    const size_t s = stats_floats(m, l, B);
    if (s > st) st = s;
  }
// ... 73 lines not shown
  if (n > m->tap_cap) return fail(m, PNVO_ERR_ARG, std::string("tap buffer too small for '") + name + "'");
  HIPCHK(m, hipMemcpyAsync(m->tap_dst, src, n * sizeof(float), hipMemcpyDeviceToDevice, s));
  return PNVO_OK;
}

}

void pnvo_drop_graphs(pnvo_handle m) {
  for (auto &g : m->graphs) {
    (void)hipGraphExecDestroy(g.exec);
    (void)hipGraphDestroy(g.graph);
  }
  m->graphs.clear();
  m->seen.clear();
}

void pnvo_chain_in_bounds(pnvo_handle h, const std::function<float(const Layer &)> &gn_bound) {
  if (h->bottleneck || h->convs.empty()) return;
  float bin = gn_bound(h->convs[0]);
  for (const Block &b : h->blocks) {
    Layer &c1 = h->convs[b.conv[0]], &c2 = h->convs[b.conv[1]];
    c1.in_bound = bin;
    c2.in_bound = gn_bound(c1);
    float skip = bin;
    if (b.ds >= 0) {
      h->convs[b.ds].in_bound = bin;
      skip = gn_bound(h->convs[b.ds]);
    }
    bin = gn_bound(c2) + skip;
  }
  h->convs[h->comp].in_bound = bin;
}

bool pnvo_conv_on_x3(pnvo_handle m, const Layer &l, int B) {
  if (!x3_layer(m, l) || l.groups <= 0) return false;
  ConvX3Args xa;
  int mw, nw;
  size_t ldsb;
  return x3_args(m, l, B, xa, &mw, &nw, &ldsb);
}

bool pnvo_conv_takes_ds(pnvo_handle m, const Layer &c1, const Layer &cd, int B) {
  if (!m->opt.ds_fuse || m->tap_dst != nullptr || m->bottleneck) return false;
  if (c1.k != 3 || c1.kw != 3 || c1.stride != 2 || c1.pad != 1 || cd.k != 1 || cd.kw != 1 || cd.stride != 2 || cd.pad != 0) return false;
  if (c1.cinp != cd.cinp || c1.coutp != cd.coutp || c1.cout != cd.cout || c1.hout != cd.hout || c1.wout != cd.wout || c1.hin != cd.hin ||
      c1.win != cd.win || c1.cout != c1.coutp || c1.groups != cd.groups || c1.groups <= 0 || cd.host_w.empty())
    return false;
  if (!x3_layer(m, c1) || !x3_layer(m, cd) || !x3_two_pieces(m, c1) || !x3_two_pieces(m, cd)) return false;
  return pnvo_conv_on_x3(m, c1, B);
}

bool pnvo_conv_takes_tail(pnvo_handle m, const Layer &l, int B) {
  if (m->tap_dst != nullptr || !m->opt.tail) return false;
  return pnvo_conv_on_x3(m, l, B);
}

namespace {
double conv_flops(const Layer &l, int B) { return 2.0 * ((double)((long)B * l.hout * l.wout) * l.cout * l.cin * l.k * l.kw); }
double conv_bytes(const Layer &l, int B) {
  return 4.0 * ((double)B * l.hin * l.win * l.cin + (double)((long)B * l.hout * l.wout) * l.cout + (double)l.cout * l.cin * l.k * l.kw);
}

int x3_operand(pnvo_handle h, Layer &q, int pieces, hipStream_t s) {
  DevBuf<unsigned short> &wpk = pieces == 2 ? q.wpk_x2 : q.wpk_x3;
  unsigned long long &gen = pieces == 2 ? q.x2_gen : q.x3_gen;
  if (wpk && gen == h->weights_gen) return PNVO_OK;
  const size_t nel = (size_t)q.k * q.kw * q.cinp * q.coutp * pieces;
  if (!wpk) HIPCHK(h, wpk.alloc(nel));
  const float *dev_w = h->train ? pnvo_train_weight_ptr(h, q.name + ".weight") : nullptr;
  if (dev_w != nullptr && pieces == 2) {
    HIPCHK(h, launch_conv_x2_repack(dev_w, q.cout, q.cin, q.cinp, q.coutp, q.k, q.kw, pnvo_train_x2_scale(h, q.name + ".weight"), wpk, s));
  } else if (dev_w != nullptr) {
    HIPCHK(h, launch_conv_x3_repack(dev_w, q.cout, q.cin, q.cinp, q.coutp, q.k, q.kw, 0, wpk, s));
  } else {
    std::vector<unsigned short> pk(nel);
    if (pieces == 2)
      q.x2_oscale = pack_conv_x2_weight(q.host_w.data(), q.cout, q.cin, q.cinp, q.coutp, q.k, q.kw, pk.data());
    else
      pack_conv_x3_weight(q.host_w.data(), q.cout, q.cin, q.cinp, q.coutp, q.k, q.kw, pk.data());
    HIPCHK(h, hipMemcpyAsync(wpk, pk.data(), nel * 2, hipMemcpyHostToDevice, s));
    HIPCHK(h, hipStreamSynchronize(s));
  }
  gen = h->weights_gen;
  return PNVO_OK;
}

int run_conv_x3(pnvo_handle m, const Layer &l, int B, const ConvRequest &r, ConvX3Args &xa, bool rows, int x3_mode, int mw, int nw,
                size_t ldsb) {
  hipStream_t s = r.s;
  const DsRide *ride = r.ride;
  const bool two = xa.np == 2;
  Layer &lm = const_cast<Layer &>(l);
  if (int rc = x3_operand(m, lm, xa.np, s)) return rc;
  if (ride != nullptr) {
    if (rows || !two || l.stride != 2 || l.k != 3) return fail(m, PNVO_ERR_STATE, "downsample ride on a conv that cannot carry it (" + l.name + ")");
    Layer &dm = const_cast<Layer &>(*ride->cd);
    if (int rc = x3_operand(m, dm, 2, s)) return rc;
    xa.ds_wpk = dm.wpk_x2;
    xa.ds_oscale = dm.x2_oscale;
    if (m->train != nullptr) {
      const float *sp = pnvo_train_x2_scale(m, dm.name + ".weight");
      xa.ds_oscale_ptr = sp ? sp + 1 : nullptr;
    }
    xa.ds_y = ride->y;
    xa.ds_stats = m->stats_ds;
  }
  GnGroup gg{0x7fffffff, 0x7fffffff, {nullptr, nullptr}, {nullptr, nullptr}}, ggd = gg;
  if (r.grp != nullptr) {
    const GroupedFwd &g = *r.grp;
    if (!two || rows) return fail(m, PNVO_ERR_STATE, "grouped forward: layer " + l.name + " is not on the float16-piece tile kernel");
    const size_t idx = (size_t)(&l - m->convs.data());
    if (idx >= m->convs.size()) return fail(m, PNVO_ERR_STATE, "grouped forward: layer outside the conv list");
    xa.grp_end0 = g.end[0];
    xa.grp_end1 = g.n > 2 ? g.end[1] : 0;
    gg.end0 = ggd.end0 = g.end[0];
    if (g.n > 2) gg.end1 = ggd.end1 = g.end[1];
    for (int k = 1; k < g.n; ++k) {
      pnvo_handle hk = g.h[k];
      Layer &lk = hk->convs[idx];
      if (!x3_two_pieces(hk, lk)) return fail(m, PNVO_ERR_STATE, "grouped forward: a model's " + l.name + " left the float16-piece form");
      if (int rc = x3_operand(hk, lk, 2, s)) return fail(m, rc, hk->err);
      xa.wpk_g[k - 1] = lk.wpk_x2;
      xa.oscale_g[k - 1] = lk.x2_oscale;
      xa.gn_gamma_g[k - 1] = gg.gamma[k - 1] = lk.gamma;
      xa.gn_beta_g[k - 1] = gg.beta[k - 1] = lk.beta;
      if (ride != nullptr) {
        const size_t idd = (size_t)(ride->cd - m->convs.data());
        Layer &dk = hk->convs[idd];
        if (!x3_two_pieces(hk, dk)) return fail(m, PNVO_ERR_STATE, "grouped forward: a model's downsample conv left the float16-piece form");
        if (int rc = x3_operand(hk, dk, 2, s)) return fail(m, rc, hk->err);
        xa.ds_wpk_g[k - 1] = dk.wpk_x2;
        xa.ds_oscale_g[k - 1] = dk.x2_oscale;
        xa.ds_gamma_g[k - 1] = ggd.gamma[k - 1] = dk.gamma;
        xa.ds_beta_g[k - 1] = ggd.beta[k - 1] = dk.beta;
      }
    }
  }
  xa.x = r.x;
  xa.wpk = two ? lm.wpk_x2 : lm.wpk_x3;
  xa.oscale = lm.x2_oscale;
  if (two && m->train != nullptr) {
    const float *sp = pnvo_train_x2_scale(m, l.name + ".weight");
    xa.oscale_ptr = sp ? sp + 1 : nullptr;
  }
  xa.y = r.y;
  xa.in_scale = r.in_scale;
  xa.in_shift = r.in_shift;
  xa.stats = m->stats;
  if (r.tail != nullptr) {
    if (r.in_scale == nullptr) return fail(m, PNVO_ERR_STATE, "block tail without the conv's GroupNorm scale/shift");
    xa.xout = r.tail->out;
  }
  const long P = (long)l.hout * l.wout;
  const int cpg = l.groups > 0 ? l.cout / l.groups : 0;
  const bool fuse = m->opt.gn_fuse && xa.slots == 1 && l.cout == l.coutp && cpg >= 1 && cpg <= 32 &&
                    32 % cpg == 0 && l.cout % cpg == 0 && (rows || !(xa.persist_wgs > 0 && l.cin == 32 && l.coutp == 32));
  if (fuse && ride != nullptr) {
    xa.ds_gamma = ride->cd->gamma;
    xa.ds_beta = ride->cd->beta;
    xa.ds_scale = ride->ss[0];
    xa.ds_shift = ride->ss[1];
    xa.ds_mu = ride->mu;
    xa.ds_rstd = ride->rstd;
  }
  if (fuse) {
    xa.gn_gamma = l.gamma;
    xa.gn_beta = l.beta;
    xa.gn_scale = r.ss[0];
    xa.gn_shift = r.ss[1];
    xa.gn_mu = r.mu;
    xa.gn_rstd = r.rstd;
    xa.gn_cpg = cpg;
    xa.gn_eps = 1e-5f;
    xa.gn_P = P;
  }
  {
    Timed t(m, s, "conv:" + l.name, conv_flops(l, B), conv_bytes(l, B) + (r.tail ? 8.0 * B * l.hin * l.win * l.cin : 0.0));
    if (rows)
      HIPCHK(m, launch_conv_rows32(xa, x3_mode, m->num_cus, s));
    else
      HIPCHK(m, launch_conv_x3(xa, l.k, l.stride, x3_mode, mw, nw, ldsb, s));
  }
  if (fuse) return PNVO_OK;
  Timed t(m, s, "gn_finalize", 0.0, 0.0);
  if (ride != nullptr) {
    const float *st2[2] = {m->stats, m->stats_ds}, *ga2[2] = {l.gamma, ride->cd->gamma}, *be2[2] = {l.beta, ride->cd->beta};
    float *sc2[2] = {r.ss[0], ride->ss[0]}, *sh2[2] = {r.ss[1], ride->ss[1]};
    float *mu2[2] = {r.mu, ride->mu}, *rs2[2] = {r.rstd, ride->rstd};
    HIPCHK(m, launch_gn_finalize_pair(st2, B, xa.slots, l.coutp, l.cout, l.groups, P, ga2, be2, 1e-5f, sc2, sh2, mu2, rs2, s,
                                      r.grp ? &gg : nullptr, r.grp ? &ggd : nullptr));
    return PNVO_OK;
  }
  HIPCHK(m, launch_gn_finalize(m->stats, B, xa.slots, l.coutp, l.cout, l.groups, P, 1, l.gamma, l.beta, 1e-5f, r.ss[0], r.ss[1], s,
                               xa.slots, r.mu, r.rstd, r.grp ? &gg : nullptr));
  return PNVO_OK;
}

int run_conv_fp32(pnvo_handle m, const Layer &l, int B, const ConvRequest &r) {
  hipStream_t s = r.s;
  ConvArgs a;
  conv_geometry(l, B, r.y_cstride, a);
  if (r.src != nullptr) {
    const int nsrc[4] = {m->cfg.n_rgb, m->cfg.n_depth, m->cfg.n_dd, m->cfg.n_tdv};
    a.src_mode = 1;
    a.zero_page = m->zero_page;
    for (int j = 0; j < m->CP / 8; ++j)
      for (int hh = 0; hh < 2; ++hh)
        for (int q = 0; q < 2; ++q) {
          const int nc = 8 * j + 4 * hh + 2 * q;
          const int tn = m->stem_tensor_of_new[nc];
          SrcPiece &pc = a.pieces[j][hh][q];
          pc.base = tn >= 0 ? r.src[tn] : nullptr;
          pc.nch = tn >= 0 ? nsrc[tn] : 0;
          pc.choff = m->stem_ch_of_new[nc];
        }
  }
  a.x = r.x;
  a.wpk = l.wpk;
  a.y = r.y;
  a.in_scale = r.in_scale;
  a.in_shift = r.in_shift;
  a.stats = r.ss ? m->stats : nullptr;
  a.bias = r.bias;
  a.bias_row = r.bias_row;
  a.relu_out = r.relu_out;
  const long P = (long)l.hout * l.wout, M = (long)B * P;
  choose_tile(M, l.coutp, &a.MT, &a.NT);
  a.slots = conv_slots((int)P, a.MT);
  if (conv3_lds_supported(a) && m->opt.conv != 3) {
    const int nt = (l.coutp / 32) % 2 == 0 ? 2 : 1;
    a.slots = conv3_lds_slots(a);
    {
      Timed t(m, s, "conv:" + l.name, conv_flops(l, B), conv_bytes(l, B));
      HIPCHK(m, launch_conv3_lds(a, nt, s));
    }
    if (r.ss) {
      Timed t(m, s, "gn_finalize", 0.0, 0.0);
      HIPCHK(m, launch_gn_finalize(m->stats, B, a.slots, l.coutp, l.cout, l.groups, P, 1, l.gamma, l.beta, 1e-5f, r.ss[0],
                                   r.ss[1], s, a.slots, r.mu, r.rstd));
    }
    return PNVO_OK;
  }
  if (r.bias != nullptr && !r.ss) {
    a.kpart = reinterpret_cast<float *>(8);
    const int ks = conv_ksplit(a);
    a.kpart = nullptr;
    if (ks > 1) {
      const size_t need = (size_t)ks * M * r.y_cstride;
      if (need > m->kpart.size()) {
        pnvo_drop_graphs(m);
        HIPCHK(m, m->kpart.alloc(need));
      }
      a.kpart = m->kpart;
      a.ksplit = ks;
    }
  }
  {
    Timed t(m, s, "conv:" + l.name, conv_flops(l, B), conv_bytes(l, B));
    HIPCHK(m, launch_conv(a, s));
    if (a.ksplit > 1 && r.head_out != nullptr && P == 1 && r.y_cstride == l.cout) {
      HIPCHK(m, launch_ksplit_reduce_head(a, r.head_w, m->head_bias, m->cfg.out_dim, r.head_out, s));
      if (r.head_rode != nullptr) *r.head_rode = true;
    } else if (a.ksplit > 1) {
      HIPCHK(m, launch_ksplit_reduce(a, s));
    }
  }
  if (r.ss) {
    Timed t(m, s, "gn_finalize", 0.0, 0.0);
    HIPCHK(m, launch_gn_finalize(m->stats, B, a.slots, l.coutp, l.cout, l.groups, P, a.MT * 32, l.gamma, l.beta, 1e-5f,
                                 r.ss[0], r.ss[1], s, 0, r.mu, r.rstd));
  }
  return PNVO_OK;
}
}

int pnvo_run_conv(pnvo_handle m, const Layer &l, int B, const ConvRequest &r) {
  if (r.ss && r.src == nullptr && r.bias == nullptr && !r.relu_out && r.y_cstride == l.coutp && x3_layer(m, l)) {
    ConvX3Args xa;
    x3_fill(m, l, B, xa);
    if (r.tail != nullptr) {
      xa.res = r.tail->res;
      xa.res_scale = r.tail->res_scale;
      xa.res_shift = r.tail->res_shift;
    }
    const int x3_mode = r.tail ? (r.tail->res ? 2 : 3) : (r.in_scale ? 1 : 0);
    const bool rows = xa.np == 2 && m->opt.x3_rows && conv_rows32_plan(xa, l.k, l.stride, x3_mode, m->num_cus);
    int mw = 0, nw = 0;
    size_t ldsb = 0;
    if (rows || conv_x3_plan(xa, l.k, l.stride, &mw, &nw, &ldsb)) return run_conv_x3(m, l, B, r, xa, rows, x3_mode, mw, nw, ldsb);
  }
  if (r.tail != nullptr) return fail(m, PNVO_ERR_STATE, "block tail handed to a conv that cannot take it (" + l.name + ")");
  if (r.grp != nullptr && r.ss != nullptr) return fail(m, PNVO_ERR_STATE, "grouped forward: layer " + l.name + " fell off the float16-piece tile kernel");
  return run_conv_fp32(m, l, B, r);
}

StemPlan pnvo_stem_plan(pnvo_handle m, bool train_fwd, const RawFrames &raw) {
  const Layer &stem = m->convs[0];
  StemPlan p;
  p.lds_serves = (m->CPL <= 32) && (stem.coutp == 32 || stem.coutp == 64) && stem.cout == stem.coutp;
  const bool keeps_place = !m->dense_sticky || (!train_fwd && p.lds_serves);
  if (keeps_place && m->mx_ok && (!train_fwd || m->train_mx) && m->opt.stem <= 1)
    p.kernel = StemPlan::MX;
  else if (keeps_place && m->dd_ok && m->opt.stem != 3)
    p.kernel = StemPlan::DD;
  else
    p.kernel = p.lds_serves ? StemPlan::LDS : StemPlan::GENERIC;
  const bool fused = p.kernel == StemPlan::MX || p.kernel == StemPlan::DD;
  p.standin = fused && m->dense_sticky;
  p.slots = stem_slots(m, p.kernel);
  const bool on_device = m->opt.input_fallback && m->dd_flag != nullptr && !train_fwd && p.lds_serves;
  p.repairs = fused && !p.standin && raw.depth == nullptr && on_device;
  p.marks = m->dd_flag != nullptr && !m->dense_sticky && raw.depth == nullptr && !on_device;
  const bool loaded_current = m->train == nullptr || m->weights_gen == m->weights_gen_at_load;
  const bool h2_current = m->mx_wpk2_dev || (train_fwd ? m->train == nullptr : loaded_current);
  const bool want2 = train_fwd ? m->opt.train_pieces == 2 : m->opt.pieces == 2;
  p.pieces = (want2 && h2_current && m->mx_wpk2 != nullptr) ? 2 : 3;
  p.h2_from_host = m->opt.pieces == 2 && m->mx_wpk2 != nullptr && loaded_current;
  return p;
}

double pnvo_stem_in_bytes(pnvo_handle m, int B, const RawFrames &raw) {
  const pnvo_config &c = m->cfg;
  return (double)B * c.height * c.width * (raw.depth ? (c.n_rgb ? 6.0 : 0.0) + 8.0 + (c.n_tdv ? 8.0 : 0.0) : 4.0 * m->convs[0].cin);
}

void pnvo_stem_mx_input(pnvo_handle m, int B, const float *const *src, const RawFrames &raw, StemMXArgs &a) {
  for (int k = 0; k < 4; ++k) a.src[k] = src[k];
  a.zero_page = m->mx_pages;
  a.B = B;
  a.H = m->cfg.height;
  a.W = m->cfg.width;
  a.Ho = m->Hs;
  a.Wo = m->Ws;
  a.slots = stem_slots(m, StemPlan::MX);
  if (raw.depth == nullptr) return;
  a.raw_rgb = raw.rgb;
  a.raw_depth = raw.depth;
  a.raw_flags = (m->cfg.n_depth > 0 ? 1 : 0) | (m->cfg.n_dd > 0 ? 2 : 0);
  a.raw_err = raw.err;
  const int bins = 10;
  for (int i = 0; i < bins; ++i) a.edges[i] = (float)((double)i * 1.0 / (double)bins);
  a.edges[bins] = 1.0f;
  a.edges[bins + 1] = 1.0f;
  a.src[0] = a.src[1] = a.src[2] = nullptr;
}

int pnvo_launch_stem_mx(pnvo_handle m, const StemMXArgs &a, int pieces, int ntiles, bool bf16_out, const GroupedFwd *grp, hipStream_t s) {
  const int form = m->opt.stem_form;
  const bool resident = grp == nullptr && (form == 3 || form == 4 || form == 0) && stem_rs_takes(a, pieces, ntiles, bf16_out, m->num_cus);
  if (!bf16_out) m->mx_prof_rs = resident;
  if (resident)
    HIPCHK(m, launch_stem_rs(a, pieces, !bf16_out && (form == 4 || form == 0), m->num_cus, s));
  else
    HIPCHK(m, launch_stem_mx(a, pieces, ntiles, bf16_out, s));
  return PNVO_OK;
}

static void stem_lds_args(pnvo_handle m, int B, const StemRequest &r, int slots, StemArgs &a) {
  const pnvo_config &c = m->cfg;
  const int nsrc[4] = {c.n_rgb, c.n_depth, c.n_dd, c.n_tdv};
  std::memset(&a, 0, sizeof(a));
  for (int j = 0; j < m->CPL / 8; ++j)
    for (int hh = 0; hh < 2; ++hh)
      for (int q = 0; q < 2; ++q) {
        const int nc = 8 * j + 4 * hh + 2 * q;
        const int tn = nc < m->CP ? m->stem_tensor_of_new[nc] : -1;
        a.pieces[j][hh][q].base = tn >= 0 ? r.src[tn] : nullptr;
        a.pieces[j][hh][q].nch = tn >= 0 ? nsrc[tn] : 0;
        a.pieces[j][hh][q].choff = tn >= 0 ? m->stem_ch_of_new[nc] : 0;
      }
  a.sc = m->stem_sc;
  a.sh = m->stem_sh;
  a.wpk = m->stem_wpk16;
  a.zero_page = m->zero_page;
  a.y = r.y;
// ... 114 lines not shown
  a.bad_onehot = m->dd_flag_dev;
  a.y = r.y;
  a.stats = m->stats;
  a.B = B;
  a.H = c.height;
  a.W = c.width;
  a.Ho = m->Hs;
  a.Wo = m->Ws;
  a.bins = m->dd_bins;
  a.slots = p.slots;
  a.dbg = m->opt.stem_dbg;
  if (a.dbg == 9) {
    if (!m->dd_prof) {
      HIPCHK(m, m->dd_prof.alloc(8));
      HIPCHK(m, hipMemset(m->dd_prof, 0, 64));
    }
    a.prof = m->dd_prof;
  }
  Timed t = stem_timed(m, B, r, false);
  HIPCHK(m, launch_stem_dd(a, r.s));
  return PNVO_OK;
}

int pnvo_run_stem(pnvo_handle m, int B, const StemRequest &r) {
  const Layer &stem = m->convs[0];
  const StemPlan p = pnvo_stem_plan(m, r.train_fwd, r.raw);
  int rc = PNVO_OK;
  if (r.pool_keys != nullptr && !p.pools()) return fail(m, PNVO_ERR_STATE, "pooled stem output asked of a stem kernel without it");
  GnGroup sgg{0x7fffffff, 0x7fffffff, {nullptr, nullptr}, {nullptr, nullptr}};
  switch (p.kernel) {
    case StemPlan::MX: rc = stem_launch_mx(m, B, r, p, sgg); break;
    case StemPlan::DD: rc = stem_launch_dd(m, B, r, p); break;
    case StemPlan::LDS: {
      StemArgs a;
      stem_lds_args(m, B, r, p.slots, a);
      a.dbg = m->opt.stem_dbg;
      a.lds_pad = m->opt.stem_dbg_pad;
      Timed t = stem_timed(m, B, r, false);
      HIPCHK(m, launch_stem_lds(a, stem.coutp, r.s));
      break;
    }
    case StemPlan::GENERIC:
      return pnvo_run_conv(m, stem, B, {.in_scale = m->stem_sc, .in_shift = m->stem_sh, .y = r.y, .y_cstride = stem.coutp, .ss = r.ss,
                                        .mu = r.mu, .rstd = r.rstd, .src = r.src, .grp = r.grp, .s = r.s});
  }
  if (rc != PNVO_OK) return rc;
  if (p.kernel != StemPlan::LDS) {
    if (p.repairs && (rc = pnvo_stem_standin(m, B, r, p.slots, m->dd_flag_dev)) != PNVO_OK) return rc;
    if ((rc = pnvo_mark_stem(m, r.s, p)) != PNVO_OK) return rc;
  }
  if (r.slots_out != nullptr) *r.slots_out = p.slots;
  if (!r.skip_finalize) {
    Timed t(m, r.s, "gn_finalize", 0.0, 0.0);
    HIPCHK(m, launch_gn_finalize(m->stats, B, p.slots, stem.coutp, stem.cout, stem.groups, (long)m->Hs * m->Ws, 1, stem.gamma, stem.beta,
                                 1e-5f, r.ss[0], r.ss[1], r.s, p.slots, r.mu, r.rstd, r.grp ? &sgg : nullptr));
  }
  return PNVO_OK;
}

int pnvo_ensure_workspace(pnvo_handle m, int B) { return ensure_workspace(m, B); }

namespace {
struct OptChoice {
  const char *word;
  int value;
};
struct OptDef {
  const char *key, *env;
  int PnvoOptions::*field;
  bool numeric;
  OptChoice choices[7];
};
const OptDef kOptions[] = {
    {"stem", "PNVO_STEM", &PnvoOptions::stem, false, {{"auto", 0}, {"mx", 1}, {"dd", 2}, {"dense", 3}, {nullptr, 0}}},
    {"conv", "PNVO_CONV", &PnvoOptions::conv, false, {{"auto", 0}, {"x3", 1}, {"fp32", 2}, {"generic", 3}, {nullptr, 0}}},
    {"pieces", "PNVO_PIECES", &PnvoOptions::pieces, false, {{"2", 2}, {"3", 3}, {nullptr, 0}}},
    {"stem_form", "PNVO_STEM_FORM", &PnvoOptions::stem_form, false, {{"auto", 0}, {"tiles", 2}, {"resident", 3}, {"fast", 4}, {nullptr, 0}}},
    {"train_pieces", "PNVO_TRAIN_PIECES", &PnvoOptions::train_pieces, false, {{"2", 2}, {"3", 3}, {nullptr, 0}}},
    {"x3_persist", "PNVO_X3_PERSIST", &PnvoOptions::x3_persist, false, {{"on", 1}, {"off", 0}, {nullptr, 0}}},
    {"x3_rows", "PNVO_X3_ROWS", &PnvoOptions::x3_rows, false, {{"on", 1}, {"off", 0}, {nullptr, 0}}},
    {"x3_strip", "PNVO_X3_STRIP", &PnvoOptions::x3_strip, false, {{"on", 1}, {"off", 0}, {nullptr, 0}}},
    {"x3_fine", "PNVO_X3_FINE", &PnvoOptions::x3_fine, false, {{"on", 1}, {"off", 0}, {nullptr, 0}}},
    {"x3_w8", "PNVO_X3_W8", &PnvoOptions::x3_w8, false, {{"on", 1}, {"off", 0}, {nullptr, 0}}},
    {"x3_ksplit", "PNVO_X3_KSPLIT", &PnvoOptions::x3_ksplit, false, {{"on", 1}, {"off", 0}, {nullptr, 0}}},
    {"fc_rows", "PNVO_FC_ROWS", &PnvoOptions::fc_rows, true, {{nullptr, 0}}},
    {"head_fuse", "PNVO_HEAD_FUSE", &PnvoOptions::head_fuse, false, {{"on", 1}, {"off", 0}, {nullptr, 0}}},
    {"ds_fuse", "PNVO_DS_FUSE", &PnvoOptions::ds_fuse, false, {{"on", 1}, {"off", 0}, {nullptr, 0}}},
    {"gn_fuse", "PNVO_GN_FUSE", &PnvoOptions::gn_fuse, false, {{"on", 1}, {"off", 0}, {nullptr, 0}}},
    {"x3_s2", nullptr, &PnvoOptions::x3_s2, false, {{"on", 1}, {"off", 0}, {nullptr, 0}}},
    {"tail", "PNVO_TAIL", &PnvoOptions::tail, false, {{"fused", 1}, {"separate", 0}, {nullptr, 0}}},
    {"pool", "PNVO_POOL", &PnvoOptions::pool, false, {{"fused", 1}, {"separate", 0}, {nullptr, 0}}},
    {"graph", "PNVO_GRAPH", &PnvoOptions::graph, true, {{nullptr, 0}}},
    {"stem_dbg", nullptr, &PnvoOptions::stem_dbg, true, {{nullptr, 0}}},
    {"stem_dbg_pad", nullptr, &PnvoOptions::stem_dbg_pad, true, {{nullptr, 0}}},
    {"wgrad_stem", "PNVO_WGRAD_STEM", &PnvoOptions::wgrad_stem, false, {{"mx", 0}, {"fp32", 1}, {nullptr, 0}}},
    {"wgrad3", "PNVO_WGRAD3", &PnvoOptions::wgrad3, false, {{"x3", 1}, {"fp32", 0}, {nullptr, 0}}},
    {"pool_bwd", "PNVO_POOL_BWD", &PnvoOptions::pool_bwd, false, {{"fused", 1}, {"separate", 0}, {nullptr, 0}}},
    {"dgrad", "PNVO_DGRAD", &PnvoOptions::dgrad, false, {{"phase", 1}, {"masked", 0}, {nullptr, 0}}},
    {"bf16_fuse", nullptr, &PnvoOptions::bf16_fuse, false, {{"on", 1}, {"off", 0}, {nullptr, 0}}},
    {"input_fallback", "PNVO_INPUT_FALLBACK", &PnvoOptions::input_fallback, false, {{"on", 1}, {"off", 0}, {nullptr, 0}}},
    {"small_net", "PNVO_SMALL_NET", &PnvoOptions::small_net, false, {{"on", 1}, {"off", 0}, {nullptr, 0}}},
    {"small_max", "PNVO_SMALL_MAX", &PnvoOptions::small_max, true, {{nullptr, 0}}},
    {"small_coop", "PNVO_SMALL_COOP", &PnvoOptions::small_coop, true, {{nullptr, 0}}},
    {"small_prof", "PNVO_SMALL_PROF", &PnvoOptions::small_prof, true, {{nullptr, 0}}},
};

const OptDef *find_option(const char *key) {
  for (const OptDef &d : kOptions)
    if (std::strcmp(d.key, key) == 0) return &d;
  return nullptr;
}

bool parse_option(const OptDef &d, const char *word, int *out) {
  if (d.numeric) {
    char *end = nullptr;
    const long v = std::strtol(word, &end, 10);
    if (end == word || *end != 0) return false;
    *out = (int)v;
    return true;
  }
  for (const OptChoice *c = d.choices; c->word != nullptr; ++c)
    if (std::strcmp(c->word, word) == 0) {
      *out = c->value;
      return true;
    }
  return false;
}

void env_defaults(pnvo_model_s *m) {
  for (const OptDef &d : kOptions) {
    const char *e = d.env ? std::getenv(d.env) : nullptr;
    int v;
    if (e && parse_option(d, e, &v)) m->opt.*(d.field) = v;
  }
  if (std::getenv("PNVO_X3_S2_OFF")) m->opt.x3_s2 = 0;
  if (std::getenv("PNVO_BF16_NOFUSE")) m->opt.bf16_fuse = 0;
  if (const char *e = std::getenv("PNVO_STEM_DBG")) std::sscanf(e, "%d,%d", &m->opt.stem_dbg, &m->opt.stem_dbg_pad);
}
}


int pnvo_input_fallback(pnvo_handle m, hipStream_t s, bool *rerun) {
  *rerun = false;
  if (!m->stem_ev_pending) return PNVO_OK;
  m->stem_ev_pending = false;
  HIPCHK(m, hipEventSynchronize(m->stem_ev));
  if (!m->dd_flag || *(volatile int *)m->dd_flag == 0) return PNVO_OK;
  *(volatile int *)m->dd_flag = 0;
  HIPCHK(m, hipMemsetAsync(m->dd_flag_dev, 0, sizeof(int), s));
  m->dense_sticky = true;
  m->fallback_count += 1;
  pnvo_drop_graphs(m);
  m->note = "note: observation values outside the fused stems' contract (fractional rgb or depth codes that are not one-hot) — "
           "the forward was re-run on the dense fp32 stem and this handle stays on it";
  *rerun = true;
  return PNVO_OK;
}

namespace {
int forward_dispatch(pnvo_handle m, int B, const FwdRequest &r);
int forward_body(pnvo_handle m, int B, const FwdRequest &r);
}


extern "C" {

#include "src_hash.h"
const char *pnvo_version(void) { return "pnvo 0.3 (gfx950: fp32 + f16/bf16 MFMA) src:" PNVO_SRC_HASH; }

const char *pnvo_last_error(pnvo_handle h) { return h ? h->err.c_str() : g_err.c_str(); }

// ... 392 lines not shown
  if (m->precision == 1) {
    pnvo_handle hs[1] = {m};
    float *outs[1] = {out};
    return pnvo_forward_bf16(hs, 1, B, r, outs);
  }
  int rc = ensure_workspace(m, B);
  if (rc != PNVO_OK) return rc;
  if ((rc = forward_dispatch(m, B, r)) != PNVO_OK) return rc;
  bool rerun = false;
  if ((rc = pnvo_input_fallback(m, r.s, &rerun)) != PNVO_OK) return rc;
  return rerun ? forward_dispatch(m, B, r) : PNVO_OK;
}

namespace {
int forward_dispatch(pnvo_handle m, int B, const FwdRequest &r) {
  const pnvo_config &c = m->cfg;
  hipStream_t s = r.s;
  int rc = PNVO_OK;
  {
    m->graph_mode = m->opt.graph;
  }
  const bool plain = !m->graph_mode || m->timing || m->tap_dst != nullptr || m->train != nullptr || m->opt.stem_dbg != 0;
  if (plain) return forward_body(m, B, r);

  const void *key[8] = {r.src[0], r.src[1], r.src[2], r.src[3], r.actions, r.raw.rgb, r.raw.depth, r.raw.err};
  const StemPlan sp = pnvo_stem_plan(m, false, r.raw);
  const size_t out_bytes = (size_t)B * c.out_dim * sizeof(float);
  for (auto &g : m->graphs)
    if (g.B == B && std::memcmp(g.key, key, sizeof(key)) == 0) {
      g.stamp = ++m->graph_clock;
      HIPCHK(m, hipGraphLaunch(g.exec, s));
      HIPCHK(m, hipMemcpyAsync(r.out, m->out_ws, out_bytes, hipMemcpyDeviceToDevice, s));
      return pnvo_mark_stem(m, s, sp);
    }
  bool again = false;
  for (auto &g : m->seen) again = again || (g.B == B && std::memcmp(g.key, key, sizeof(key)) == 0);
  if (!again) {
    pnvo_model_s::GraphEntry sn;
    std::memset(&sn, 0, sizeof(sn));
    std::memcpy(sn.key, key, sizeof(key));
    sn.B = B;
    if (m->seen.size() >= 16) m->seen.erase(m->seen.begin());
    m->seen.push_back(sn);
    return forward_body(m, B, r);
  }
  if (!m->cap_stream) HIPCHK(m, hipStreamCreateWithFlags(&m->cap_stream, hipStreamNonBlocking));
  pnvo_model_s::GraphEntry g;
  std::memcpy(g.key, key, sizeof(key));
  g.B = B;
  g.stamp = ++m->graph_clock;
  HIPCHK(m, hipStreamBeginCapture(m->cap_stream, hipStreamCaptureModeRelaxed));
  FwdRequest rcap = r;
  rcap.out = m->out_ws;
  rcap.s = m->cap_stream;
  rc = forward_body(m, B, rcap);
  const hipError_t ce = hipStreamEndCapture(m->cap_stream, &g.graph);
  if (rc != PNVO_OK) {
    if (ce == hipSuccess && g.graph) (void)hipGraphDestroy(g.graph);
    return rc;
  }
  HIPCHK(m, ce);
  HIPCHK(m, hipGraphInstantiate(&g.exec, g.graph, nullptr, nullptr, 0));
  if (m->graphs.size() >= 8) {
    size_t old = 0;
    for (size_t k = 1; k < m->graphs.size(); ++k)
      if (m->graphs[k].stamp < m->graphs[old].stamp) old = k;
    (void)hipGraphExecDestroy(m->graphs[old].exec);
    (void)hipGraphDestroy(m->graphs[old].graph);
    m->graphs.erase(m->graphs.begin() + (long)old);
  }
  m->graphs.push_back(g);
  HIPCHK(m, hipGraphLaunch(g.exec, s));
  HIPCHK(m, hipMemcpyAsync(r.out, m->out_ws, out_bytes, hipMemcpyDeviceToDevice, s));
  return pnvo_mark_stem(m, s, sp);
}
}

namespace {
int run_fc_head(pnvo_handle m, int B, const float *comp_raw, const float *sc, const float *sh, const FwdRequest &r);
bool fc_rows_usable(pnvo_handle m, int B, const FwdRequest &r);
int run_fc_rows(pnvo_handle m, pnvo_handle const *grp, const int *end, int ng, int B, const float *comp_raw, const float *sc, const float *sh,
                const FwdRequest &r);

int forward_body(pnvo_handle m, int B, const FwdRequest &r) {
  const pnvo_config &c = m->cfg;
  const GroupedFwd *grp = r.grp;
  hipStream_t s = r.s;
  int rc = PNVO_OK;
  if (m->tap_dst != nullptr && m->tap_name == "input") {
    AssembleArgs a;
    for (int k = 0; k < 4; ++k) a.src[k] = r.src[k];
    a.nsrc[0] = c.n_rgb;
    a.nsrc[1] = c.n_depth;
    a.nsrc[2] = c.n_dd;
    a.nsrc[3] = c.n_tdv;
    a.mean = c.normalize ? m->mean.data() : nullptr;
    a.stdev = m->stdev.data();
    a.C = m->C;
    a.CP = m->CP;
    a.npix = (long)B * c.height * c.width;
    HIPCHK(m, m->xin.alloc((size_t)a.npix * m->CP));
    a.out = m->xin;
    HIPCHK(m, launch_assemble(a, s));
    if ((rc = maybe_tap(m, "input", m->xin, (size_t)B * c.height * c.width * m->CP, s)) != PNVO_OK) return rc;
  }
  const Layer &stem = m->convs[0];
  float *cur = m->bufY[0], *nxt = m->bufY[1];
  const StemPlan sp = pnvo_stem_plan(m, false, r.raw);
  const bool pool_fused = !m->bottleneck && sp.pools() && m->opt.pool && stem.coutp == stem.cout &&
                          pnvo_conv_takes_tail(m, m->convs[m->blocks[0].conv[0]], B);
  const bool small = !pool_fused && sp.writes_slots() && !r.stop_after_compression && pnvo_small_usable(m, B);
  StemRequest sr{.src = {r.src[0], r.src[1], r.src[2], r.src[3]}, .raw = r.raw, .y = m->stem_raw, .ss = m->ssA, .grp = grp, .s = s};
  if (small) {
    int stem_slots = 0;
    sr.slots_out = &stem_slots;
    sr.skip_finalize = true;
    if ((rc = pnvo_run_stem(m, B, sr)) != PNVO_OK) return rc;
    return pnvo_small_forward(m, B, r, stem_slots);
  }
  if (pool_fused) {
    Timed t(m, s, "pool_init", 0.0, 4.0 * B * m->Hp * m->Wp * stem.coutp);
    HIPCHK(m, hipMemsetD32Async(reinterpret_cast<hipDeviceptr_t>(nxt), STEM_POOL_INIT, (size_t)B * m->Hp * m->Wp * stem.coutp, s));
    sr.pool_keys = reinterpret_cast<int *>(nxt);
  }
  if ((rc = pnvo_run_stem(m, B, sr)) != PNVO_OK) return rc;
  if ((rc = maybe_tap(m, "stem_conv", m->stem_raw, (size_t)B * m->Hs * m->Ws * stem.coutp, s)) != PNVO_OK) return rc;
  if (!pool_fused) {
    Timed t(m, s, "gn_relu_maxpool", 0.0, 4.0 * B * ((double)m->Hs * m->Ws + (double)m->Hp * m->Wp) * stem.coutp);
    HIPCHK(m, launch_gn_relu_maxpool(m->stem_raw, m->ssA[0], m->ssA[1], B, m->Hs, m->Ws, stem.coutp, cur, s));
  }
  if ((rc = maybe_tap(m, "maxpool", cur, (size_t)B * m->Hp * m->Wp * stem.coutp, s)) != PNVO_OK) return rc;

  BlockTail tail{};
  bool have_tail = false, have_keys = pool_fused;
  for (size_t bk = 0; bk < m->blocks.size(); ++bk) {
    const Block &b = m->blocks[bk];
    const bool ds = b.ds >= 0;
    if (m->bottleneck) {
      const Layer &b1 = m->convs[b.conv[0]];
      const Layer &b2 = m->convs[b.conv[1]];
      const Layer &b3 = m->convs[b.conv[2]];
      if ((rc = pnvo_run_conv(m, b1, B, {.x = cur, .y = m->rawA, .y_cstride = b1.coutp, .ss = m->ssA, .grp = grp, .s = s})) != PNVO_OK ||
          (rc = pnvo_run_conv(m, b2, B, {.x = m->rawA, .in_scale = m->ssA[0], .in_shift = m->ssA[1], .y = m->rawC, .y_cstride = b2.coutp,
                                         .ss = m->ssB, .grp = grp, .s = s})) != PNVO_OK ||
          (rc = pnvo_run_conv(m, b3, B, {.x = m->rawC, .in_scale = m->ssB[0], .in_shift = m->ssB[1], .y = m->rawB, .y_cstride = b3.coutp,
                                         .ss = m->ssA, .grp = grp, .s = s})) != PNVO_OK)
        return rc;
      const long Pb = (long)b3.hout * b3.wout;
      if (ds) {
        const Layer &cd = m->convs[b.ds];
        if ((rc = pnvo_run_conv(m, cd, B, {.x = cur, .y = m->rawD, .y_cstride = cd.coutp, .ss = m->ssD, .grp = grp, .s = s})) != PNVO_OK)
          return rc;
        Timed t(m, s, "residual", 0.0, 12.0 * B * Pb * b3.coutp);
        HIPCHK(m, launch_residual(m->rawB, m->ssA[0], m->ssA[1], m->rawD, m->ssD[0], m->ssD[1], B, Pb, b3.coutp, nxt, s));
      } else {
        Timed t(m, s, "residual", 0.0, 12.0 * B * Pb * b3.coutp);
        HIPCHK(m, launch_residual(m->rawB, m->ssA[0], m->ssA[1], cur, nullptr, nullptr, B, Pb, b3.coutp, nxt, s));
      }
      std::swap(cur, nxt);
      if ((rc = maybe_tap(m, b.tap.c_str(), cur, (size_t)B * Pb * b3.coutp, s)) != PNVO_OK) return rc;
      continue;
    }
    const Layer &c1 = m->convs[b.conv[0]];
    const Layer &c2 = m->convs[b.conv[1]];
    const bool ds_ride = ds && !have_keys && pnvo_conv_takes_ds(m, c1, m->convs[b.ds], B);
    const DsRide ride{ds_ride ? &m->convs[b.ds] : nullptr, m->rawD, m->ssD, nullptr, nullptr};
    if (have_keys) {
      BlockTail ktail{nullptr, nullptr, nullptr, cur};
      if ((rc = pnvo_run_conv(m, c1, B, {.x = nxt, .in_scale = m->ssA[0], .in_shift = m->ssA[1], .y = m->rawA, .y_cstride = c1.coutp,
                                         .ss = m->ssA, .tail = &ktail, .grp = grp, .s = s})) != PNVO_OK)
        return rc;
      have_keys = false;
    } else if (have_tail) {
      if (ds_ride) tail.out = nullptr;
      if ((rc = pnvo_run_conv(m, c1, B, {.x = m->rawB, .in_scale = m->ssB[0], .in_shift = m->ssB[1], .y = m->rawA, .y_cstride = c1.coutp,
                                         .ss = m->ssA, .tail = &tail, .ride = ds_ride ? &ride : nullptr, .grp = grp, .s = s})) != PNVO_OK)
        return rc;
      std::swap(cur, nxt);
      have_tail = false;
    } else if ((rc = pnvo_run_conv(m, c1, B, {.x = cur, .y = m->rawA, .y_cstride = c1.coutp, .ss = m->ssA, .ride = ds_ride ? &ride : nullptr,
                                              .grp = grp, .s = s})) != PNVO_OK) {
      return rc;
    }
    const long P = (long)c2.hout * c2.wout;
    const bool c2_small_generic = !layer_on_lds(m, c2, nullptr) && !pnvo_conv_on_x3(m, c2, B) && (size_t)B * P * c2.cinp * 4 <= ((size_t)48 << 20);
    if (c2_small_generic) {
      float *napp = ds_ride ? nxt : m->rawD;
      {
        Timed t(m, s, "gn_relu_apply", 0.0, 8.0 * B * P * c2.cinp);
        HIPCHK(m, launch_apply_ss_relu(m->rawA, m->ssA[0], m->ssA[1], B, P, c2.cinp, napp, s));
      }
      if ((rc = pnvo_run_conv(m, c2, B, {.x = napp, .y = m->rawB, .y_cstride = c2.coutp, .ss = m->ssB, .grp = grp, .s = s})) != PNVO_OK)
        return rc;
    } else if ((rc = pnvo_run_conv(m, c2, B, {.x = m->rawA, .in_scale = m->ssA[0], .in_shift = m->ssA[1], .y = m->rawB, .y_cstride = c2.coutp,
                                              .ss = m->ssB, .grp = grp, .s = s})) != PNVO_OK) {
      return rc;
    }
    if (ds) {
      const Layer &cd = m->convs[b.ds];
      if (!ds_ride &&
          (rc = pnvo_run_conv(m, cd, B, {.x = cur, .y = m->rawD, .y_cstride = cd.coutp, .ss = m->ssD, .grp = grp, .s = s})) != PNVO_OK)
        return rc;
    }
    if (pnvo_conv_takes_tail(m, m->convs[m->next_conv_after(bk)], B)) {
      tail.res = ds ? m->rawD : cur;
      tail.res_scale = ds ? m->ssD[0] : nullptr;
      tail.res_shift = ds ? m->ssD[1] : nullptr;
      tail.out = nxt;
      have_tail = true;
      continue;
    }
    {
      Timed t(m, s, "residual", 0.0, 12.0 * B * P * c2.coutp);
      HIPCHK(m, launch_residual(m->rawB, m->ssB[0], m->ssB[1], ds ? m->rawD : cur, ds ? m->ssD[0] : nullptr, ds ? m->ssD[1] : nullptr, B,
                                P, c2.coutp, nxt, s));
    }
    std::swap(cur, nxt);
    if ((rc = maybe_tap(m, b.tap.c_str(), cur, (size_t)B * P * c2.coutp, s)) != PNVO_OK) return rc;
  }

  const Layer &comp = m->convs[m->comp];
  if (have_tail) {
    tail.out = nullptr;
    if ((rc = pnvo_run_conv(m, comp, B, {.x = m->rawB, .in_scale = m->ssB[0], .in_shift = m->ssB[1], .y = m->comp_raw, .y_cstride = comp.coutp,
                                         .ss = m->ssC, .tail = &tail, .grp = grp, .s = s})) != PNVO_OK)
      return rc;
    have_tail = false;
  } else if ((rc = pnvo_run_conv(m, comp, B, {.x = cur, .y = m->comp_raw, .y_cstride = comp.coutp, .ss = m->ssC, .grp = grp, .s = s})) != PNVO_OK) {
    return rc;
  }
  if (m->tap_dst != nullptr && m->tap_name == "compression") {
    HIPCHK(m, launch_apply_ss_relu(m->comp_raw, m->ssC[0], m->ssC[1], B, (long)m->fh * m->fw, m->comp_cp, m->tapbuf, s));
    if ((rc = maybe_tap(m, "compression", m->tapbuf, (size_t)B * m->fh * m->fw * m->comp_cp, s)) != PNVO_OK) return rc;
  }
  if (r.stop_after_compression) return PNVO_OK;
  if (grp != nullptr) {
    bool rows_ok = !c.act_embed;
    FwdRequest rk = r;
    rk.actions = nullptr;
    for (int k = 0; k < grp->n; ++k) rows_ok = rows_ok && fc_rows_usable(grp->h[k], B, rk);
    if (rows_ok) return run_fc_rows(m, grp->h, grp->end, grp->n, B, m->comp_raw, m->ssC[0], m->ssC[1], rk);
    int start = 0;
    for (int k = 0; k < grp->n; ++k) {
      const int Bk = grp->end[k] - start;
      pnvo_handle hk = grp->h[k];
      if (k > 0 && (rc = ensure_workspace(hk, Bk)) != PNVO_OK) return fail(m, rc, std::string("grouped forward: ") + pnvo_last_error(hk));
      const size_t crow = (size_t)m->fh * m->fw * m->comp_cp;
      rk.out = r.out + (size_t)start * c.out_dim;
      rc = run_fc_head(hk, Bk, m->comp_raw + start * crow, m->ssC[0] + (size_t)start * m->comp_cp, m->ssC[1] + (size_t)start * m->comp_cp, rk);
      if (rc != PNVO_OK) return k > 0 ? fail(m, rc, std::string("grouped forward: ") + pnvo_last_error(hk)) : rc;
      start = grp->end[k];
    }
    return PNVO_OK;
  }
  return run_fc_head(m, B, m->comp_raw, m->ssC[0], m->ssC[1], r);
}

bool fc_rows_usable(pnvo_handle m, int B, const FwdRequest &r) {
  const long kp = (long)m->fh * m->fw * m->comp_cp;
  return m->opt.fc_rows >= B && B >= 1 && m->fc_rows_w != nullptr && m->train == nullptr && m->precision == 0 && m->opt.conv == 0 &&
         m->comp_cp > 0 && 256 % m->comp_cp == 0 && kp % 4 == 0 && kp / 4 <= 64L * FC_ROWS_MAXV && m->cfg.hidden % 4 == 0 &&
         (r.features_only || m->head_w_plain != nullptr);
}

int run_fc_rows(pnvo_handle m, pnvo_handle const *grp, const int *end, int ng, int B, const float *comp_raw, const float *sc, const float *sh,
                const FwdRequest &r) {
  const pnvo_config &c = m->cfg;
  FcRowsArgs a;
  std::memset(&a, 0, sizeof(a));
  a.x = comp_raw;
  a.sc = sc;
  a.sh = sh;
  a.hid = r.features_only ? r.out : m->hid;
  a.out = r.out;
  a.actions = c.act_embed ? r.actions : nullptr;
  a.B = B;
  a.Kp = m->fh * m->fw * m->comp_cp;
  a.cp = m->comp_cp;
  a.hidden = c.hidden;
  a.out_dim = c.out_dim;
  a.ngroups = ng;
  for (int k = 0; k < ng; ++k) {
    a.end[k] = end[k];
    a.w[k] = grp[k]->fc_rows_w;
    a.bias[k] = grp[k]->fc_bias;
    a.head_w[k] = grp[k]->head_w_plain;
    a.head_b[k] = grp[k]->head_bias;
  }
  Timed t(m, r.s, "conv:" + m->fc.name, 2.0 * B * (double)a.Kp * c.hidden, 4.0 * ng * (double)a.Kp * c.hidden);
  HIPCHK(m, launch_fc_rows(a, !r.features_only, r.s));
  return PNVO_OK;
}

int run_fc_head(pnvo_handle m, int B, const float *comp_raw, const float *sc, const float *sh, const FwdRequest &r) {
  const pnvo_config &c = m->cfg;
  float *out = r.out;
  hipStream_t s = r.s;
  int rc = PNVO_OK;
  if (fc_rows_usable(m, B, r)) {
    pnvo_handle one[1] = {m};
    const int end[1] = {B};
    if ((rc = run_fc_rows(m, one, end, 1, B, comp_raw, sc, sh, r)) != PNVO_OK) return rc;
    return r.features_only ? PNVO_OK : maybe_tap(m, "hidden", m->hid, (size_t)B * c.hidden, s);
  }
  bool head_rode = false;
  const float *head_w = m->train != nullptr ? pnvo_train_weight_ptr(m, "output_head.1.weight") : m->head_w_plain;
  float *head_out = (m->opt.head_fuse && !r.features_only && c.out_dim <= 4 && head_w != nullptr) ? out : nullptr;
  if ((rc = pnvo_run_conv(m, m->fc, B, {.x = comp_raw, .in_scale = sc, .in_shift = sh, .y = m->hid, .y_cstride = c.hidden, .bias = m->fc_bias,
                                        .bias_row = c.act_embed ? r.actions : nullptr, .relu_out = 1, .head_w = head_w, .head_out = head_out,
                                        .head_rode = &head_rode, .s = s})) != PNVO_OK)
    return rc;
  if ((rc = maybe_tap(m, "hidden", m->hid, (size_t)B * c.hidden, s)) != PNVO_OK) return rc;
  if (head_rode) return PNVO_OK;
// ... 411 lines not shown
  }
  if (m->dd_prof) {
    unsigned long long pr[8] = {0, 0, 0, 0, 0, 0, 0, 0};
    (void)hipMemcpy(pr, m->dd_prof, 64, hipMemcpyDeviceToHost);
    const double nt_ = (double)(pr[3] ? pr[3] : 1);
    std::fprintf(stderr, "[pnvo] stem_dd phases (cycles per tile, workgroup thread 0): staging %.0f  k-loop %.0f (of which "
                 "row barriers %.0f)  epilogue %.0f  (%llu tiles)\n", (double)pr[0] / nt_, (double)pr[1] / nt_,
                 (double)pr[4] / nt_, (double)pr[2] / nt_, pr[3]);
  }
  for (auto &r : m->trecs) {
    (void)hipEventDestroy(r.a);
    (void)hipEventDestroy(r.b);
  }
  for (auto e : m->evpool) (void)hipEventDestroy(e);
  delete m;
  return PNVO_OK;
}

int pnvo_set_tap(pnvo_handle h, const char *name, float *dst, size_t capacity) {
  if (!h) return fail(h, PNVO_ERR_ARG, "null handle");
  h->tap_name = name ? name : "";
  h->tap_dst = name ? dst : nullptr;
  h->tap_cap = capacity;
  return PNVO_OK;
}

int pnvo_tap_shape(pnvo_handle h, const char *name, int B, int64_t shape[4]) {
  if (!h || !name || !shape) return fail(h, PNVO_ERR_ARG, "null argument");
  const pnvo_config &c = h->cfg;
  const std::string n = name;
  auto set = [&](int64_t a, int64_t b, int64_t cc, int64_t d) {
    shape[0] = a;
    shape[1] = b;
    shape[2] = cc;
    shape[3] = d;
    return PNVO_OK;
  };
  if (n == "input") return set(B, c.height, c.width, h->CP);
  if (n == "stem_conv") return set(B, h->Hs, h->Ws, c.baseplanes);
  if (n == "maxpool") return set(B, h->Hp, h->Wp, c.baseplanes);
  if (n == "compression") return set(B, h->fh, h->fw, h->comp_cp);
  if (n == "hidden") return set(B, 1, 1, c.hidden);
  for (const Block &b : h->blocks)
    if (n == b.tap) return set(B, h->last(b).hout, h->last(b).wout, h->last(b).coutp);
  return fail(h, PNVO_ERR_ARG, "unknown tap '" + n + "'");
}

int pnvo_layer_kernel(pnvo_handle h, const char *name, int B, char *family, size_t cap, double *executed_flops) {
  if (!h || !name || !family || cap == 0 || B <= 0) return fail(h, PNVO_ERR_ARG, "bad argument");
  for (size_t li = 1; li < h->convs.size(); ++li) {
    const Layer &l = h->convs[li];
    if (l.name != name) continue;
    const double alg = 2.0 * B * l.hout * l.wout * (double)l.cout * l.cin * l.k * l.kw;
    if (pnvo_stem_plan(h, false, {}).writes_slots() && pnvo_small_usable(h, B)) {
      std::snprintf(family, cap, "smallnet");
      if (executed_flops) {
        const int mb = l.cinp >= 128 ? 1 : l.cinp >= 64 ? 2 : 4, th = mb == 4 ? 8 : 4, tw = mb == 1 ? 4 : 8;
        *executed_flops = 2.0 * B * ((l.hout + th - 1) / th) * ((l.wout + tw - 1) / tw) * (th * tw) * (double)rup(l.cout, 16) * l.cinp * l.k * l.kw;
      }
      return PNVO_OK;
    }
    ConvX3Args xa;
    int mw, nw;
    size_t ldsb;
    const Layer *c1 = l.block >= 0 && h->blocks[l.block].ds == (int)li ? &h->convs[h->blocks[l.block].conv[0]] : nullptr;
    if (c1 && pnvo_conv_takes_ds(h, *c1, l, B) && x3_args(h, *c1, B, xa, &mw, &nw, &ldsb)) {
      std::snprintf(family, cap, "x2-rides");
      if (executed_flops) *executed_flops = 3.0 * 2.0 * (double)B * xa.tiles_r * xa.tiles_c * xa.MT * 32.0 * l.coutp * (double)l.cinp;
      return PNVO_OK;
    }
    if (x3_layer(h, l) && l.groups > 0 && x3_args(h, l, B, xa, &mw, &nw, &ldsb)) {
      std::snprintf(family, cap, xa.np == 2 ? "x2" : "x3");
      if (executed_flops)
        *executed_flops = (xa.np == 2 ? 3.0 : 6.0) * 2.0 * (double)B * xa.tiles_r * xa.tiles_c * xa.MT * 32.0 * l.coutp * (double)l.cinp * l.k * l.kw;
      return PNVO_OK;
    }
    std::snprintf(family, cap, "%s", layer_on_lds(h, l, nullptr) ? "fp32-lds" : "fp32-generic");
    if (executed_flops) *executed_flops = alg;
    return PNVO_OK;
  }
  return fail(h, PNVO_ERR_ARG, std::string("no residual-stage conv named '") + name + "'");
}

int pnvo_timing_mode(pnvo_handle h, int mode) {
  if (!h) return fail(h, PNVO_ERR_ARG, "null handle");
  h->timing = mode ? 1 : 0;
  return PNVO_OK;
}

int pnvo_timing_read(pnvo_handle h, pnvo_kernel_time *entries, int cap, int *n_out) {
  if (!h || !n_out) return fail(h, PNVO_ERR_ARG, "null argument");
  for (auto &r : h->trecs) {
    HIPCHK(h, hipEventSynchronize(r.b));
    float ms = 0.f;
    HIPCHK(h, hipEventElapsedTime(&ms, r.a, r.b));
    h->tentries[r.entry].total_ms += ms;
    h->evpool.push_back(r.a);
    h->evpool.push_back(r.b);
  }
  h->trecs.clear();
  const int n = (int)h->tentries.size();
  *n_out = n;
  for (int k = 0; k < n && k < cap && entries; ++k) entries[k] = h->tentries[k];
  h->tentries.clear();
  h->tindex.clear();
  return PNVO_OK;
}

size_t pnvo_packed_conv_floats(int cout, int cin, int kh, int kw) { return packed_conv_floats(cout, cin, kh, kw); }

int pnvo_pack_conv_weight(const float *oihw, int cout, int cin, int kh, int kw, float *out) {
  if (!oihw || !out || cout <= 0 || cin <= 0 || kh <= 0 || kw <= 0) return fail(nullptr, PNVO_ERR_ARG, "bad argument");
  pack_conv_weight(oihw, cout, cin, kh, kw, out);
  return PNVO_OK;
}

}
```

pointnav-vo_amd/csrc/pnvo_model.h:

```cpp
#pragma once
#include <hip/hip_runtime.h>

#include <map>
#include <functional>
#include <string>
#include <vector>

#include "../../include/pnvo.h"
#include "pnvo_internal.h"
#include "dev_buf.h"

using pnvo::DevBuf;
using pnvo::DevPair;

static inline int rup(int x, int m) { return (x + m - 1) / m * m; }
static inline int halve(int x) { return (x - 1) / 2 + 1; }

struct Layer {
  std::string name, gn;
  int cin = 0, cinp = 0, cout = 0, coutp = 0, k = 1, kw = 1, stride = 1, pad = 0;
  int hin = 0, win = 0, hout = 0, wout = 0, groups = 1;
  DevBuf<float> wpk, gamma, beta;
  std::vector<float> host_w;
  DevBuf<unsigned short> wpk_x3;
  unsigned long long x3_gen = 0;
  DevBuf<unsigned short> wpk_x2;
  unsigned long long x2_gen = 0;
  float x2_oscale = 1.f;
  float in_bound = 3.0e38f;
  int block = -1;
};

struct Block {
  int stage = 0, index = 0;
  int nconv = 0;
  int conv[3] = {-1, -1, -1};
  int ds = -1;
  std::string tap;
};

struct PnvoOptions {
  int stem = 0;
  int conv = 0;
  int stem_form = 0;
  int pieces = 2;
  int train_pieces = 2;
  int x3_rows = 1;
  int x3_persist = 1;
  int x3_strip = 1;
  int x3_fine = 1;
  int x3_w8 = 1;
  int x3_ksplit = 1;
  int fc_rows = 48;
  int head_fuse = 1;
  int ds_fuse = 1;
  int gn_fuse = 1;
  int x3_s2 = 1;
  int tail = 1;
  int pool = 1;
  int graph = 0;
  int stem_dbg = 0, stem_dbg_pad = 0;
  int wgrad_stem = 0;
  int wgrad3 = 1;
  int pool_bwd = 1;
  int dgrad = 1;
  int bf16_fuse = 1;
  int input_fallback = 1;
  int small_net = 1;
  int small_max = 3;
  int small_prof = 0;
  int small_coop = 1;
};

struct TimingRec {
  hipEvent_t a, b;
  int entry;
};

struct pnvo_model_s {
  pnvo_config cfg;
  int device = 0;
  std::string err;
  std::string note;
  bool loaded = false;

  int C = 0, CP = 0;
  int Hs = 0, Ws = 0, Hp = 0, Wp = 0, fh = 0, fw = 0, comp_c = 0, comp_cp = 0;
  std::vector<Layer> convs;
  std::vector<Block> blocks;
  int comp = -1;
  const Layer &last(const Block &b) const { return convs[b.conv[b.nconv - 1]]; }
  int next_conv_after(size_t k) const { return k + 1 < blocks.size() ? blocks[k + 1].conv[0] : comp; }
  Layer fc, head;
  DevBuf<float> fc_bias, head_bias;
  DevBuf<float> fc_rows_w;
  DevBuf<float> head_w_plain;
  std::vector<float> mean, stdev;
  std::vector<int> stem_ref_of_new;
  std::vector<int> stem_tensor_of_new, stem_ch_of_new;
  DevBuf<float> stem_sc, stem_sh, zero_page;
  DevBuf<float> kpart;
  DevBuf<float> stem_wpk16;
  int CPL = 0;
  bool dd_ok = false;
  int dd_bins = 0;
  std::vector<int> dd_dense_tensor, dd_dense_ch;
  DevBuf<float> dd_wpk, dd_table, dd_sc, dd_sh;
  DevBuf<int> dd_flag;
  DevBuf<int> dd_flag_dev;
  DevBuf<unsigned long long> dd_prof;

  bool mx_ok = false;
  DevBuf<unsigned short> mx_wpk3;
  DevBuf<unsigned short> mx_wpk2;
  float mx_oscale = 1.f;
  DevBuf<float> mx_scale2_dev;
  bool mx_wpk2_dev = false;
  std::vector<float> mx_wk, mx_wk_swapped;
  int mx_xslot[4] = {-1, -1, -1, -1};
  std::vector<int> mx_slot_ref, mx_slot_new;
  DevBuf<float> mx_pages;
  DevBuf<unsigned long long> mx_prof;
  bool mx_prof_rs = false;
  int num_cus = 256;
  bool train_mx = false;
  PnvoOptions opt;
  bool dense_sticky = false;
  int fallback_count = 0;
  DevBuf<float> stats_ds;
  hipEvent_t stem_ev = nullptr;
  bool stem_ev_pending = false;
  DevBuf<float> rawws[3];
  int rawws_cap = 0;
  int precision = 0;
  unsigned long long load_gen = 0;
  unsigned long long weights_gen_at_load = 0;
  unsigned long long uid = 0;
  unsigned long long weights_gen = 0;
  void *bf = nullptr;

  int cap = 0;
  DevBuf<float> xin, stem_raw, bufY[2];
  DevBuf<float> rawA, rawB, rawD, rawC, comp_raw, hid, stats;
  bool bottleneck = false;
  DevPair<float> ssA, ssB, ssD, ssC;
  DevBuf<float> tapbuf;

  std::string tap_name;
  float *tap_dst = nullptr;
  size_t tap_cap = 0;

  void *train = nullptr;
  void *small = nullptr;

  struct GraphEntry {
    const void *key[8];
    int B;
    hipGraph_t graph;
    hipGraphExec_t exec;
    unsigned long long stamp;
  };
  std::vector<GraphEntry> graphs;
  std::vector<GraphEntry> seen;
  DevBuf<float> out_ws;
  hipStream_t cap_stream = nullptr;
  int graph_mode = -1;
  unsigned long long graph_clock = 0;

  int timing = 0;
  std::vector<pnvo_kernel_time> tentries;
  std::map<std::string, int> tindex;
  std::vector<TimingRec> trecs;
  std::vector<hipEvent_t> evpool;
};


struct BlockTail {
  const float *res, *res_scale, *res_shift;
  float *out;
};

struct DsRide {
  const Layer *cd;
  float *y;
  float *const *ss;
  float *mu, *rstd;
};

struct GroupedFwd {
  int n;
  pnvo_model_s *h[3];
  int end[3];
};

struct ConvRequest {
  const float *x = nullptr;
  const float *in_scale = nullptr, *in_shift = nullptr;
  float *y = nullptr;
  int y_cstride = 0;
  float *const *ss = nullptr;
  float *mu = nullptr, *rstd = nullptr;
  const float *bias = nullptr;
  const int64_t *bias_row = nullptr;
  int relu_out = 0;
  const float *const *src = nullptr;
  const BlockTail *tail = nullptr;
  const DsRide *ride = nullptr;
  const GroupedFwd *grp = nullptr;
  const float *head_w = nullptr;
  float *head_out = nullptr;
  bool *head_rode = nullptr;
  hipStream_t s = nullptr;
};

struct RawFrames {
  const unsigned char *rgb = nullptr;
  const float *depth = nullptr;
  int *err = nullptr;
};

struct StemPlan {
  enum Kernel { MX, DD, LDS, GENERIC } kernel = GENERIC;
  bool lds_serves = false;
  bool standin = false;
  bool repairs = false;
  bool marks = false;
  int pieces = 3;
  bool h2_from_host = false;
  int slots = 0;
  bool writes_slots() const { return kernel != GENERIC; }
  bool pools() const { return kernel == MX; }
  bool raw_stager() const { return kernel == MX && !standin; }
};

struct StemRequest {
  const float *src[4] = {nullptr, nullptr, nullptr, nullptr};
  RawFrames raw;
  float *y = nullptr;
  float *const *ss = nullptr;
  float *mu = nullptr, *rstd = nullptr;
  int *pool_keys = nullptr;
  bool train_fwd = false;
  int *slots_out = nullptr;
  bool skip_finalize = false;
  const GroupedFwd *grp = nullptr;
  hipStream_t s = nullptr;
};

struct FwdRequest {
  const float *src[4] = {nullptr, nullptr, nullptr, nullptr};
  RawFrames raw;
  const int64_t *actions = nullptr;
  float *out = nullptr;
  bool features_only = false;
  bool stop_after_compression = false;
  const GroupedFwd *grp = nullptr;
  hipStream_t s = nullptr;
};

int pnvo_run_conv(pnvo_handle m, const Layer &l, int B, const ConvRequest &r);
bool pnvo_conv_takes_ds(pnvo_handle m, const Layer &c1, const Layer &cd, int B);
bool pnvo_conv_on_x3(pnvo_handle m, const Layer &l, int B);
bool pnvo_conv_takes_tail(pnvo_handle m, const Layer &l, int B);
void pnvo_pack_conv_weight_cinp(const float *oihw, int cout, int cin, int cinp, int kh, int kw, std::vector<float> &out);
StemPlan pnvo_stem_plan(pnvo_handle m, bool train_fwd, const RawFrames &raw);
int pnvo_run_stem(pnvo_handle m, int B, const StemRequest &r);
void pnvo_stem_mx_input(pnvo_handle m, int B, const float *const *src, const RawFrames &raw, pnvo::StemMXArgs &a);
double pnvo_stem_in_bytes(pnvo_handle m, int B, const RawFrames &raw);
int pnvo_launch_stem_mx(pnvo_handle m, const pnvo::StemMXArgs &a, int pieces, int ntiles, bool bf16_out, const GroupedFwd *grp, hipStream_t s);
int pnvo_mark_stem(pnvo_handle m, hipStream_t s, const StemPlan &p);
int pnvo_input_fallback(pnvo_handle m, hipStream_t s, bool *rerun);
void pnvo_train_free(pnvo_handle m);
const float *pnvo_train_weight_ptr(pnvo_handle m, const std::string &name);
int pnvo_forward_compression(pnvo_handle m, const float *depth, int B, void *stream);
const float *pnvo_train_hidden(pnvo_handle m);
int pnvo_train_backward_from_hidden(pnvo_handle m, const float *dh, bool stop_after_fc, void *stream);
void pnvo_chain_in_bounds(pnvo_handle h, const std::function<float(const Layer &)> &gn_bound);
const float *pnvo_train_x2_scale(pnvo_handle m, const std::string &name);
void pnvo_bf16_free(pnvo_handle m);
bool pnvo_small_usable(pnvo_handle m, int B);
int pnvo_small_forward(pnvo_handle m, int B, const FwdRequest &r, int stem_slots);
void pnvo_small_free(pnvo_handle m);
int pnvo_forward_bf16(pnvo_handle *hs, int nm, int B, const FwdRequest &r, float *const *outs);
int pnvo_fail(pnvo_handle h, int code, const std::string &msg);
int pnvo_ensure_workspace(pnvo_handle m, int B);
void pnvo_drop_graphs(pnvo_handle m);

#define HIPCHK(h, expr)                                                                                   \
  do {                                                                                                    \
    hipError_t e__ = (expr);                                                                              \
    if (e__ != hipSuccess)                                                                                \
      return pnvo_fail(h, PNVO_ERR_HIP, std::string(#expr) + ": " + hipGetErrorString(e__));             \
  } while (0)

struct PnvoTimed {
  pnvo_model_s *m;
  hipStream_t s;
  int rec = -1;
  PnvoTimed(pnvo_model_s *m_, hipStream_t s_, const std::string &name, double flops, double bytes);
  ~PnvoTimed();
};
```

pointnav-vo_amd/vo_cnn.py:

```python
import ctypes as C
import math

import torch
import torch.nn as nn

from . import _lib
from . import model_spec as ms
from .common_vars import DEFAULT_DELTA_STATE_SIZE, N_ACTS, TOP_DOWN_VIEW_PAIR_CHANNEL
from .registry import baseline_registry


class _Holder(nn.Module):
    """Anonymous container so dotted state_dict names resolve exactly as in the reference module tree."""


def _init_tensor(name, shape, fan_in=None):
    t = torch.empty(shape)
    if len(shape) == 4 or (len(shape) == 2 and name != "action_embedding.weight"):
        if name == "output_head.1.weight":
            nn.init.orthogonal_(t)
        else:
            nn.init.kaiming_uniform_(t, a=math.sqrt(5))
    elif name == "action_embedding.weight":
        nn.init.normal_(t)
# ... 183 lines not shown
                raise TypeError("forward() missing required argument 'actions' (act_embed model)")
            a = actions.to(device=dev, dtype=torch.int64).contiguous().reshape(-1)
            keep.append(a)
            act_ptr = C.c_void_p(a.data_ptr())
        out = torch.empty((B, c.out_dim), device=dev, dtype=torch.float32)
        with torch.cuda.device(dev):
            stream = torch.cuda.current_stream(dev).cuda_stream
            _lib.check(_lib.lib.pnvo_forward(self._handle, ptrs[0], ptrs[1], ptrs[2], ptrs[3], act_ptr, int(B),
                                             C.c_void_p(out.data_ptr()), C.c_void_p(stream)), self._handle)
        return out

    def forward_raw(self, rgb_frames, depth_frames, top_down_view=None, actions=None, err_flag=None):
        if self.training:
            raise RuntimeError("forward_raw is the eval-mode forward (train-mode forwards take observation pairs)")
        ref = self._ref_param()
        if ref.device.type != "cuda":
            raise RuntimeError("pointnav_vo_amd VO models run on an MI355X only (there is no CPU fallback)")
        dev = ref.device
        self._ensure_handle(dev)
        self._sync_weights()
        c = self.cfg
        B = depth_frames.shape[0]
        keep = []

        def ptr(t, dtype, shape, what):
            if t is None:
                return None
            if t.device != dev or t.dtype != dtype or tuple(t.shape) != shape:
                raise ValueError(f"{what}: expected {dtype} {shape} on {dev}, got {t.dtype} {tuple(t.shape)} on {t.device}")
            t = t.contiguous()
            keep.append(t)
            return C.c_void_p(t.data_ptr())

        p_rgb = ptr(rgb_frames if c.n_rgb else None, torch.uint8, (B, 2, c.height, c.width, 3), "rgb_frames")
        p_dep = ptr(depth_frames, torch.float32, (B, 2, c.height, c.width), "depth_frames")
        p_tdv = ptr(top_down_view if c.n_tdv else None, torch.float32, (B, c.height, c.width, 2), "top_down_view")
        if c.n_rgb and p_rgb is None:
            raise ValueError("this model has the rgb modality: rgb_frames is required")
        if c.n_tdv and p_tdv is None:
            raise ValueError("this model has the top_down_view modality: top_down_view is required")
        act_ptr = None
        if c.act_embed:
            if actions is None:
                raise TypeError("forward_raw() missing required argument 'actions' (act_embed model)")
            a = actions.to(device=dev, dtype=torch.int64).contiguous().reshape(-1)
            keep.append(a)
            act_ptr = C.c_void_p(a.data_ptr())
        out = torch.empty((B, c.out_dim), device=dev, dtype=torch.float32)
        with torch.cuda.device(dev):
            stream = torch.cuda.current_stream(dev).cuda_stream
            _lib.check(_lib.lib.pnvo_forward_raw(self._handle, p_rgb, p_dep, p_tdv, act_ptr, int(B), C.c_void_p(out.data_ptr()),
                                                 C.c_void_p(err_flag.data_ptr()) if err_flag is not None else None,
                                                 C.c_void_p(stream)), self._handle)
        return out

    def tap(self, name, observation_pairs, actions=None):
        dev = next(self.parameters()).device
        self._ensure_handle(dev)
        first = next(v for v in observation_pairs.values())
        B = first.shape[0]
        shape = (C.c_int64 * 4)()
        _lib.check(_lib.lib.pnvo_tap_shape(self._handle, name.encode(), int(B), shape), self._handle)
        buf = torch.empty(tuple(int(s) for s in shape), device=dev, dtype=torch.float32)
        _lib.check(_lib.lib.pnvo_set_tap(self._handle, name.encode(), C.c_void_p(buf.data_ptr()), buf.numel()),
                   self._handle)
        try:
            out = self.forward(observation_pairs, actions)
        finally:
            _lib.lib.pnvo_set_tap(self._handle, None, None, 0)
        return out, buf

    def check_inputs(self):
        if self._handle is not None:
            _lib.check(_lib.lib.pnvo_check_inputs(self._handle), self._handle)

    def layer_kernel(self, name, batch):
        dev = next(self.parameters()).device
        self._ensure_handle(dev)
        self._sync_weights()
        buf, fl = C.create_string_buffer(32), C.c_double(0.0)
        _lib.check(_lib.lib.pnvo_layer_kernel(self._handle, name.encode(), int(batch), buf, 32, C.byref(fl)), self._handle)
        return buf.value.decode(), float(fl.value)

    def timing(self, enable):
        dev = next(self.parameters()).device
        self._ensure_handle(dev)
        _lib.check(_lib.lib.pnvo_timing_mode(self._handle, int(bool(enable))), self._handle)

    def timing_read(self):
        ent = (_lib.pnvo_kernel_time * 128)()
        n = C.c_int(0)
        _lib.check(_lib.lib.pnvo_timing_read(self._handle, ent, 128, C.byref(n)), self._handle)
        return [dict(name=ent[i].name.decode(), launches=int(ent[i].launches), total_ms=float(ent[i].total_ms),
                     flops=float(ent[i].flops), bytes=float(ent[i].bytes)) for i in range(min(n.value, 128))]


def _obs_ptrs(model, observation_pairs, dev):
    c = model.cfg
    ptrs, B, keep = [], None, []
    for key, n in (("rgb", c.n_rgb), ("depth", c.n_depth), ("discretized_depth", c.n_dd), ("top_down_view", c.n_tdv)):
        if n == 0:
            ptrs.append(None)
            continue
        t = observation_pairs[key]
        if t.device != dev:
            raise RuntimeError(f"observation '{key}' is on {t.device}, model on {dev}")
        t = t.to(torch.float32).contiguous()
        if t.dim() != 4 or t.shape[1] != c.height or t.shape[2] != c.width or t.shape[3] != n:
            raise ValueError(f"observation '{key}' has shape {tuple(t.shape)}, expected [B,{c.height},{c.width},{n}]")
        B = t.shape[0] if B is None else B
        assert t.shape[0] == B
        keep.append(t)
        ptrs.append(C.c_void_p(t.data_ptr()))
    return ptrs, B, keep


def dual_forward(model_a, model_b, observation_pairs):
    ref = next(model_a.parameters())
    if ref.device.type != "cuda" or next(model_b.parameters()).device != ref.device:
        raise RuntimeError("dual_forward: both models must be on the same MI355X (there is no CPU fallback)")
    if model_a.training or model_b.training:
        raise RuntimeError("dual_forward is the eval-mode forward of both models")
    dev = ref.device
    for m in (model_a, model_b):
        m._ensure_handle(dev)
        m._sync_weights()
    ptrs, B, keep = _obs_ptrs(model_a, observation_pairs, dev)
    oa = torch.empty((B, model_a.cfg.out_dim), device=dev, dtype=torch.float32)
    ob = torch.empty_like(oa)
    with torch.cuda.device(dev):
        stream = torch.cuda.current_stream(dev).cuda_stream
        _lib.check(_lib.lib.pnvo_forward_dual(model_a._handle, model_b._handle, ptrs[0], ptrs[1], ptrs[2], ptrs[3], int(B),
                                              C.c_void_p(oa.data_ptr()), C.c_void_p(ob.data_ptr()), C.c_void_p(stream)),
                   model_a._handle)
    return oa, ob


def dual_forward_raw(model_a, model_b, rgb_frames, depth_frames, top_down_view=None, err_flag=None):
    ref = next(model_a.parameters())
    if ref.device.type != "cuda" or next(model_b.parameters()).device != ref.device:
        raise RuntimeError("dual_forward_raw: both models must be on the same MI355X (there is no CPU fallback)")
    if model_a.training or model_b.training:
        raise RuntimeError("dual_forward_raw is the eval-mode forward of both models")
    dev = ref.device
    for m in (model_a, model_b):
        m._ensure_handle(dev)
        m._sync_weights()
    c = model_a.cfg
    B = depth_frames.shape[0]
    rgb = rgb_frames.contiguous() if c.n_rgb else None
    dep = depth_frames.contiguous()
    tdv = top_down_view.contiguous() if c.n_tdv else None
    assert dep.dtype == torch.float32 and tuple(dep.shape) == (B, 2, c.height, c.width) and dep.device == dev
    assert rgb is None or (rgb.dtype == torch.uint8 and tuple(rgb.shape) == (B, 2, c.height, c.width, 3) and rgb.device == dev)
    assert tdv is None or (tdv.dtype == torch.float32 and tuple(tdv.shape) == (B, c.height, c.width, 2) and tdv.device == dev)
    oa = torch.empty((B, c.out_dim), device=dev, dtype=torch.float32)
    ob = torch.empty_like(oa)
    p = lambda t: C.c_void_p(t.data_ptr()) if t is not None else None
    with torch.cuda.device(dev):
        stream = torch.cuda.current_stream(dev).cuda_stream
        _lib.check(_lib.lib.pnvo_forward_dual_raw(model_a._handle, model_b._handle, p(rgb), p(dep), p(tdv), int(B), p(oa), p(ob),
                                                  p(err_flag), C.c_void_p(stream)), model_a._handle)
    return oa, ob


def grouped_supported(models):
# ... 96 lines not shown
```

Before: 113,100.

## Chain consecutive residual-block convs into single multi-phase kernels

New measurement: 112,200. About the same (-0.9%).

```diff
diff --git a/include/pnvo.h b/include/pnvo.h
--- a/include/pnvo.h
+++ b/include/pnvo.h
@@ -235,6 +235,8 @@
 
 int pnvo_layer_kernel(pnvo_handle h, const char *name, int B, char *family, size_t cap, double *executed_flops);
 
+int pnvo_last_chains(pnvo_handle h, char *buf, size_t cap);
+
 int pnvo_timing_mode(pnvo_handle h, int mode);
 int pnvo_timing_read(pnvo_handle h, pnvo_kernel_time *entries, int cap, int *n_out);
 
diff --git a/pointnav-vo_amd/_lib.py b/pointnav-vo_amd/_lib.py
--- a/pointnav-vo_amd/_lib.py
+++ b/pointnav-vo_amd/_lib.py
@@ -124,6 +124,7 @@
     "pnvo_rollout_gather_frames": (C.c_int, [C.c_void_p, C.c_void_p, C.c_int, C.c_int64] + [C.c_int] * 3 + [C.c_void_p, C.c_void_p]),
     "pnvo_avgpool2": (C.c_int, [C.c_void_p, C.c_int, C.c_int, C.c_int, C.c_void_p, C.c_void_p]),
     "pnvo_layer_kernel": (C.c_int, [C.c_void_p, C.c_char_p, C.c_int, C.c_char_p, C.c_size_t, C.POINTER(C.c_double)]),
+    "pnvo_last_chains": (C.c_int, [C.c_void_p, C.c_char_p, C.c_size_t]),
     "pnvo_timing_mode": (C.c_int, [C.c_void_p, C.c_int]),
     "pnvo_timing_read": (C.c_int, [C.c_void_p, C.POINTER(pnvo_kernel_time), C.c_int, C.POINTER(C.c_int)]),
     "pnvo_packed_conv_floats": (C.c_size_t, [C.c_int, C.c_int, C.c_int, C.c_int]),
diff --git a/pointnav-vo_amd/csrc/conv_chain.h b/pointnav-vo_amd/csrc/conv_chain.h
--- /dev/null
+++ b/pointnav-vo_amd/csrc/conv_chain.h
@@ -0,0 +1,27 @@
+#pragma once
+#include "pnvo_internal.h"
+
+namespace pnvo {
+
+constexpr int CONV_CHAIN_MAX = 4;
+
+constexpr int CHAIN_DSF = 8;
+constexpr int CHAIN_M5 = 16;
+
+int conv_rows32_chain_match(const int *modes, int n);
+int conv_x3_chain_match(const int *kinds, int n);
+bool conv_rows32_chainable(const ConvX3Args &a);
+bool conv_x3_chainable(const ConvX3Args &a, int ks, int stride, int mode, int mw, int nw, int *kind);
+hipError_t launch_conv_rows32_chain(const ConvX3Args *a, const int *modes, int n, int num_cus, hipStream_t s);
+hipError_t launch_conv_x3_chain(const ConvX3Args *a, const int *kinds, int n, size_t lds_bytes, hipStream_t s);
+
+#if defined(__HIPCC__)
+__device__ __forceinline__ void conv_chain_fence() {
+  asm volatile("s_waitcnt vmcnt(0)" ::: "memory");
+  __builtin_amdgcn_fence(__ATOMIC_RELEASE, "workgroup");
+  __builtin_amdgcn_s_barrier();
+  __builtin_amdgcn_fence(__ATOMIC_ACQUIRE, "agent");
+}
+#endif
+
+}
diff --git a/pointnav-vo_amd/csrc/conv_rows.hip b/pointnav-vo_amd/csrc/conv_rows.hip
--- a/pointnav-vo_amd/csrc/conv_rows.hip
+++ b/pointnav-vo_amd/csrc/conv_rows.hip
@@ -1,6 +1,7 @@
 #include <cstdio>
 #include <cstdlib>
 
+#include "conv_chain.h"
 #include "pnvo_internal.h"
 
 namespace pnvo {
@@ -45,7 +46,7 @@
 }
 
 template <int MODE>
-__global__ __launch_bounds__(RS_THREADS) __attribute__((amdgpu_waves_per_eu(2, 2))) void conv_rows32_kernel(const ConvX3Args p) {
+__device__ __forceinline__ void conv_rows32_body(const ConvX3Args &p) {
   extern __shared__ __attribute__((aligned(16))) unsigned char lds[];
   const int tid = (int)threadIdx.x;
   const int lane = tid & 63;
@@ -332,6 +333,21 @@
   }
 }
 
+template <int MODE>
+__global__ __launch_bounds__(RS_THREADS) __attribute__((amdgpu_waves_per_eu(2, 2))) void conv_rows32_kernel(const ConvX3Args p) {
+  conv_rows32_body<MODE>(p);
+}
+
+template <int N>
+struct RowsChainArgs {
+  ConvX3Args a[N];
+};
+template <int... MODES>
+__global__ __launch_bounds__(RS_THREADS) __attribute__((amdgpu_waves_per_eu(2, 2))) void conv_rows32_chain_kernel(const RowsChainArgs<sizeof...(MODES)> c) {
+  int k = 0;
+  ((conv_rows32_body<MODES>(c.a[k++]), conv_chain_fence()), ...);
+}
+
 bool conv_rows32_plan(ConvX3Args &a, int ks, int stride, int mode, int num_cus) {
   if (ks != 3 || stride != 1 || a.np != 2 || a.CIN != 32 || a.COUTP != 32 || a.in_absmax != nullptr) return false;
   if (mode < 0 || mode > 3 || (mode == 2 && a.res_scale != nullptr)) return false;
@@ -393,4 +409,45 @@
   return hipGetLastError();
 }
 
-}
+bool conv_rows32_chainable(const ConvX3Args &a) {
+  return a.rs_bands == 1 && a.stats != nullptr && a.gn_scale != nullptr && a.grp_end0 == 0 && a.prof == nullptr && a.rs_dbg == 0 &&
+         a.oscale_ptr == nullptr;
+}
+
+namespace {
+constexpr int RS_CHAINS[][CONV_CHAIN_MAX] = {{3, 1, 2, 1}};
+
+template <int... MODES>
+hipError_t launch_rows_chain(const ConvX3Args *a, unsigned gx, hipStream_t s) {
+  static std::mutex attr_mu;
+  static unsigned long long attr_seen = 0;
+  if (pnvo_first_launch_on_device(attr_mu, attr_seen)) {
+    const hipError_t e = hipFuncSetAttribute(reinterpret_cast<const void *>(conv_rows32_chain_kernel<MODES...>),
+                                             hipFuncAttributeMaxDynamicSharedMemorySize, RS_LDS);
+    if (e != hipSuccess) return e;
+  }
+  RowsChainArgs<sizeof...(MODES)> c;
+  for (size_t k = 0; k < sizeof...(MODES); ++k) c.a[k] = a[k];
+  hipLaunchKernelGGL((conv_rows32_chain_kernel<MODES...>), dim3(gx), dim3(RS_THREADS), RS_LDS, s, c);
+  return hipGetLastError();
+}
+}
+
+int conv_rows32_chain_match(const int *modes, int n) {
+  for (const auto &sh : RS_CHAINS) {
+    bool ok = n >= CONV_CHAIN_MAX;
+    for (int k = 0; ok && k < CONV_CHAIN_MAX; ++k) ok = modes[k] == sh[k];
+    if (ok) return CONV_CHAIN_MAX;
+  }
+  return 0;
+}
+
+hipError_t launch_conv_rows32_chain(const ConvX3Args *a, const int *modes, int n, int num_cus, hipStream_t s) {
+  if (conv_rows32_chain_match(modes, n) != n) return hipErrorInvalidValue;
+  for (int k = 0; k < n; ++k)
+    if (!conv_rows32_chainable(a[k]) || a[k].B != a[0].B) return hipErrorInvalidValue;
+  const unsigned gx = (unsigned)(a[0].B < num_cus ? a[0].B : num_cus);
+  return launch_rows_chain<3, 1, 2, 1>(a, gx, s);
+}
+
+}
diff --git a/pointnav-vo_amd/csrc/conv_x3.hip b/pointnav-vo_amd/csrc/conv_x3.hip
--- a/pointnav-vo_amd/csrc/conv_x3.hip
+++ b/pointnav-vo_amd/csrc/conv_x3.hip
@@ -3,6 +3,7 @@
 #include <cstdlib>
 #include <cstring>
 
+#include "conv_chain.h"
 #include "pnvo_internal.h"
 
 namespace pnvo {
@@ -34,7 +35,7 @@
 }
 
 template <int KS, int STRIDE, int MODE, int MW, int NW, int NP, bool DSF = false, bool W8 = false, bool KSW = false>
-__global__ __launch_bounds__(W8 ? 512 : 256) __attribute__((amdgpu_waves_per_eu(W8 ? 2 : x3_wpe(MW, NW, NP, DSF), W8 ? 2 : x3_wpe(MW, NW, NP, DSF)))) void conv_x3_kernel(const ConvX3Args p) {
+__device__ __forceinline__ void conv_x3_body(const ConvX3Args &p) {
   constexpr int NTH = W8 ? 512 : 256, NWV = NTH / 64;
   constexpr int EMW = KSW ? 1 : MW;
   static_assert(!KSW || (NW == 1 && NP == 2 && KS == 3 && !DSF && !W8), "K split over the waves: float16-piece 3x3 convs, one N-tile");
@@ -617,6 +618,30 @@
     d[3] = t_f - t_0;
     d[4] = wall_clock64() - r_0;
   }
+}
+
+template <int KS, int STRIDE, int MODE, int MW, int NW, int NP, bool DSF = false, bool W8 = false, bool KSW = false>
+__global__ __launch_bounds__(W8 ? 512 : 256) __attribute__((amdgpu_waves_per_eu(W8 ? 2 : x3_wpe(MW, NW, NP, DSF), W8 ? 2 : x3_wpe(MW, NW, NP, DSF)))) void conv_x3_kernel(const ConvX3Args p) {
+  conv_x3_body<KS, STRIDE, MODE, MW, NW, NP, DSF, W8, KSW>(p);
+}
+
+template <int N>
+struct X3ChainArgs {
+  ConvX3Args a[N];
+};
+template <int KIND>
+__device__ __forceinline__ void conv_x3_chain_phase(const ConvX3Args &p) {
+  if constexpr ((KIND & CHAIN_DSF) != 0)
+    conv_x3_body<3, 2, KIND & 7, 3, 1, 2, true, true>(p);
+  else if constexpr ((KIND & CHAIN_M5) != 0)
+    conv_x3_body<3, 1, KIND & 7, 5, 1, 2, false, true>(p);
+  else
+    conv_x3_body<3, 1, KIND, 3, 1, 2, false, true>(p);
+}
+template <int... KINDS>
+__global__ __launch_bounds__(512) __attribute__((amdgpu_waves_per_eu(2, 2))) void conv_x3_chain_kernel(const X3ChainArgs<sizeof...(KINDS)> c) {
+  int k = 0;
+  ((conv_x3_chain_phase<KINDS>(c.a[k++]), conv_chain_fence()), ...);
 }
 
 
@@ -1006,6 +1031,16 @@
   PNVO_X3(0, 1, 1) PNVO_X3(1, 1, 1) PNVO_X3(0, 2, 1) PNVO_X3(1, 2, 1) PNVO_X3(0, 2, 2) PNVO_X3(1, 2, 2) PNVO_X3(0, 3, 2) PNVO_X3(1, 3, 2)
   PNVO_X3(2, 1, 1) PNVO_X3(2, 2, 1) PNVO_X3(2, 2, 2) PNVO_X3(2, 3, 2) PNVO_X3(3, 1, 1) PNVO_X3(3, 2, 1) PNVO_X3(3, 2, 2) PNVO_X3(3, 3, 2)
 
+  if constexpr (KS == 3 && STRIDE == 1 && NP == 2) if (a.w8 && mw == 5) {
+#define PNVO_X3W5(MODE_)                                                                                               \
+  if (mode == MODE_ && nw == 1) {                                                                                      \
+    hipLaunchKernelGGL((conv_x3_kernel<KS, STRIDE, MODE_, 5, 1, NP, false, true>), grid, dim3(512), ldsb, s, a);       \
+    return hipGetLastError();                                                                                          \
+  }
+    PNVO_X3W5(0) PNVO_X3W5(1) PNVO_X3W5(2) PNVO_X3W5(3)
+#undef PNVO_X3W5
+    return hipErrorInvalidValue;
+  }
   if (KS == 3 && STRIDE == 1 && NP == 2) {
     PNVO_X3(0, 5, 1) PNVO_X3(1, 5, 1) PNVO_X3(2, 5, 1) PNVO_X3(3, 5, 1)
     if constexpr (KS == 3 && STRIDE == 1 && NP == 2) if (a.ksw) {
@@ -1077,6 +1112,7 @@
   if (!((ks == 3 && (stride == 1 || stride == 2)) || (ks == 1 && stride == 2))) return false;
   a.w8 = 0;
   a.ksw = 0;
+  const bool w8_ok = (a.w8_ok & 1) != 0, w8s_ok = (a.w8_ok & 2) != 0;
   const int ntt = a.COUTP / 32;
   int TR, TC;
   if (stride == 2 && ks == 3) {
@@ -1138,6 +1174,10 @@
     *nw = 1;
     if (*mw > 5) return false;
     if (*mw < 5) *mw = 5;
+    if (w8s_ok && a.tiles_r * a.tiles_c == 1 && a.B >= 224) {
+      a.w8 = 1;
+      a.wn = 4;
+    }
   } else if (ntt == 1) {
     a.wn = 1;
     *mw = a.CIN > 32 ? 1 : 2;
@@ -1163,7 +1203,7 @@
       a.wn = 2;
       *mw = 2;
     }
-    if (a.w8_ok && !fine && ntiles >= 200 && a.MT == 3 && ntt == 8 && a.np == 2 && ks == 3) {
+    if (w8_ok && !fine && ntiles >= 200 && a.MT == 3 && ntt == 8 && a.np == 2 && ks == 3) {
       a.w8 = 1;
       a.wn = 8;
       *mw = 3;
@@ -1247,6 +1287,49 @@
   if (ks == 3 && stride == 2) return launch_ks<3, 2, 3>(a, mode, mw, nw, grid, lds_bytes, s);
   if (ks == 1 && stride == 2) return launch_ks<1, 2, 3>(a, mode, mw, nw, grid, lds_bytes, s);
   return hipErrorInvalidValue;
+}
+
+bool conv_x3_chainable(const ConvX3Args &a, int ks, int stride, int mode, int mw, int nw, int *kind) {
+  const bool dsf = a.ds_wpk != nullptr;
+  if (!a.w8 || a.np != 2 || ks != 3 || (mw != 3 && mw != 5) || nw != 1 || a.tiles_r * a.tiles_c != 1 || a.COUTP != 32 * a.wn) return false;
+  if (mw == 5 && dsf) return false;
+  if (a.stats == nullptr || a.gn_scale == nullptr || a.grp_end0 != 0 || a.in_absmax != nullptr || a.oscale_ptr != nullptr) return false;
+  if (dsf ? (stride != 2 || (mode != 0 && mode != 2) || a.ds_scale == nullptr || a.ds_oscale_ptr != nullptr) : stride != 1) return false;
+  if (conv_x3_persistent(a, ks, stride, mode, mw, nw)) return false;
+  *kind = mode + (dsf ? CHAIN_DSF : 0) + (mw == 5 ? CHAIN_M5 : 0);
+  return true;
+}
+
+namespace {
+constexpr int X3_CHAINS[][CONV_CHAIN_MAX + 1] = {{4, CHAIN_DSF + 2, 1, 2, 1}, {3, 1, 2, 1, -1},
+                                                 {3, CHAIN_M5 + 1, CHAIN_M5 + 2, CHAIN_M5 + 1, -1}};
+
+template <int... KINDS>
+hipError_t launch_x3_chain(const ConvX3Args *a, size_t ldsb, hipStream_t s) {
+  X3ChainArgs<sizeof...(KINDS)> c;
+  for (size_t k = 0; k < sizeof...(KINDS); ++k) c.a[k] = a[k];
+  const long ntiles = a[0].B;
+  hipLaunchKernelGGL((conv_x3_chain_kernel<KINDS...>), dim3((unsigned)(((ntiles + 7) / 8) * 8)), dim3(512), ldsb, s, c);
+  return hipGetLastError();
+}
+}
+
+int conv_x3_chain_match(const int *kinds, int n) {
+  for (const auto &sh : X3_CHAINS) {
+    bool ok = n >= sh[0];
+    for (int k = 0; ok && k < sh[0]; ++k) ok = kinds[k] == sh[1 + k];
+    if (ok) return sh[0];
+  }
+  return 0;
+}
+
+hipError_t launch_conv_x3_chain(const ConvX3Args *a, const int *kinds, int n, size_t lds_bytes, hipStream_t s) {
+  if (n < 1 || conv_x3_chain_match(kinds, n) != n) return hipErrorInvalidValue;
+  for (int k = 0; k < n; ++k)
+    if (a[k].B != a[0].B || a[k].prof != nullptr) return hipErrorInvalidValue;
+  if (n == 4) return launch_x3_chain<CHAIN_DSF + 2, 1, 2, 1>(a, lds_bytes, s);
+  if (kinds[0] & CHAIN_M5) return launch_x3_chain<CHAIN_M5 + 1, CHAIN_M5 + 2, CHAIN_M5 + 1>(a, lds_bytes, s);
+  return launch_x3_chain<1, 2, 1>(a, lds_bytes, s);
 }
 
 void pack_conv_x3_weight(const float *oihw, int cout, int cin, int cinp, int coutp, int kh_, int kw_, unsigned short *out) {
diff --git a/pointnav-vo_amd/csrc/pnvo_api.hip b/pointnav-vo_amd/csrc/pnvo_api.hip
--- a/pointnav-vo_amd/csrc/pnvo_api.hip
+++ b/pointnav-vo_amd/csrc/pnvo_api.hip
@@ -13,6 +13,7 @@
 #include <thread>
 #include <vector>
 
+#include "conv_chain.h"
 #include "pnvo_model.h"
 
 using namespace pnvo;
@@ -253,7 +254,7 @@
   xa.force = m->opt.conv == 1;
   xa.strip = m->opt.x3_strip;
   xa.fine = m->opt.x3_fine;
-  xa.w8_ok = m->opt.x3_w8;
+  xa.w8_ok = (m->opt.x3_w8 ? 1 : 0) | (m->opt.x3_w8s ? 2 : 0);
   xa.ksw_ok = m->opt.x3_ksplit;
   xa.persist_wgs = m->opt.x3_persist ? 3 * m->num_cus : 0;
   xa.np = x3_two_pieces(m, l) ? 2 : 3;
@@ -493,6 +494,39 @@
     HIPCHK(h, hipStreamSynchronize(s));
   }
   gen = h->weights_gen;
+  return PNVO_OK;
+}
+
+int chain_flush(pnvo_handle m, hipStream_t s) {
+  std::vector<pnvo_model_s::ChainPending> q;
+  q.swap(m->chain_pending);
+  for (size_t i = 0; i < q.size();) {
+    ConvX3Args a[CONV_CHAIN_MAX];
+    int kinds[CONV_CHAIN_MAX];
+    const int n = (int)std::min(q.size() - i, (size_t)CONV_CHAIN_MAX);
+    for (int k = 0; k < n; ++k) {
+      a[k] = q[i + k].a;
+      kinds[k] = q[i + k].kind;
+    }
+    const pnvo_model_s::ChainPending &c = q[i];
+    const int len = c.rows ? conv_rows32_chain_match(kinds, n) : conv_x3_chain_match(kinds, n);
+    if (len >= 2) {
+      size_t ldsb = 0;
+      for (int k = 0; k < len; ++k) ldsb = std::max(ldsb, q[i + k].ldsb);
+      if (c.rows)
+        HIPCHK(m, launch_conv_rows32_chain(a, kinds, len, m->num_cus, s));
+      else
+        HIPCHK(m, launch_conv_x3_chain(a, kinds, len, ldsb, s));
+      for (int k = 0; k < len; ++k) m->chain_log += (k ? "+" : (m->chain_log.empty() ? "" : ";")) + q[i + k].layer->name;
+      i += (size_t)len;
+    } else {
+      if (c.rows)
+        HIPCHK(m, launch_conv_rows32(c.a, c.mode, m->num_cus, s));
+      else
+        HIPCHK(m, launch_conv_x3(c.a, c.ks, c.stride, c.mode, c.mw, c.nw, c.ldsb, s));
+      i += 1;
+    }
+  }
   return PNVO_OK;
 }
 
@@ -585,6 +619,14 @@
     xa.gn_eps = 1e-5f;
     xa.gn_P = P;
   }
+  int kind = x3_mode;
+  const bool link = m->chain_on && fuse && B <= m->num_cus && (rows ? conv_rows32_chainable(xa) : conv_x3_chainable(xa, l.k, l.stride, x3_mode, mw, nw, &kind));
+  if (!m->chain_pending.empty() && (!link || (m->chain_pending.back().rows != 0) != rows))
+    if (int rc = chain_flush(m, s)) return rc;
+  if (link) {
+    m->chain_pending.push_back({xa, rows ? 1 : 0, kind, l.k, l.stride, x3_mode, mw, nw, ldsb, &l});
+    return PNVO_OK;
+  }
   {
     Timed t(m, s, "conv:" + l.name, conv_flops(l, B), conv_bytes(l, B) + (r.tail ? 8.0 * B * l.hin * l.win * l.cin : 0.0));
     if (rows)
@@ -685,6 +727,8 @@
 }
 }
 
+int pnvo_chain_flush(pnvo_handle m, hipStream_t s) { return m->chain_pending.empty() ? PNVO_OK : chain_flush(m, s); }
+
 int pnvo_run_conv(pnvo_handle m, const Layer &l, int B, const ConvRequest &r) {
   if (r.ss && r.src == nullptr && r.bias == nullptr && !r.relu_out && r.y_cstride == l.coutp && x3_layer(m, l)) {
     ConvX3Args xa;
@@ -702,6 +746,7 @@
   }
   if (r.tail != nullptr) return fail(m, PNVO_ERR_STATE, "block tail handed to a conv that cannot take it (" + l.name + ")");
   if (r.grp != nullptr && r.ss != nullptr) return fail(m, PNVO_ERR_STATE, "grouped forward: layer " + l.name + " fell off the float16-piece tile kernel");
+  if (int rc = pnvo_chain_flush(m, r.s)) return rc;
   return run_conv_fp32(m, l, B, r);
 }
 
@@ -982,11 +1027,13 @@
     {"x3_strip", "PNVO_X3_STRIP", &PnvoOptions::x3_strip, false, {{"on", 1}, {"off", 0}, {nullptr, 0}}},
     {"x3_fine", "PNVO_X3_FINE", &PnvoOptions::x3_fine, false, {{"on", 1}, {"off", 0}, {nullptr, 0}}},
     {"x3_w8", "PNVO_X3_W8", &PnvoOptions::x3_w8, false, {{"on", 1}, {"off", 0}, {nullptr, 0}}},
+    {"x3_w8s", "PNVO_X3_W8S", &PnvoOptions::x3_w8s, false, {{"on", 1}, {"off", 0}, {nullptr, 0}}},
     {"x3_ksplit", "PNVO_X3_KSPLIT", &PnvoOptions::x3_ksplit, false, {{"on", 1}, {"off", 0}, {nullptr, 0}}},
     {"fc_rows", "PNVO_FC_ROWS", &PnvoOptions::fc_rows, true, {{nullptr, 0}}},
     {"head_fuse", "PNVO_HEAD_FUSE", &PnvoOptions::head_fuse, false, {{"on", 1}, {"off", 0}, {nullptr, 0}}},
     {"ds_fuse", "PNVO_DS_FUSE", &PnvoOptions::ds_fuse, false, {{"on", 1}, {"off", 0}, {nullptr, 0}}},
     {"gn_fuse", "PNVO_GN_FUSE", &PnvoOptions::gn_fuse, false, {{"on", 1}, {"off", 0}, {nullptr, 0}}},
+    {"chain", "PNVO_CHAIN", &PnvoOptions::chain, false, {{"on", 1}, {"off", 0}, {nullptr, 0}}},
     {"x3_s2", nullptr, &PnvoOptions::x3_s2, false, {{"on", 1}, {"off", 0}, {nullptr, 0}}},
     {"tail", "PNVO_TAIL", &PnvoOptions::tail, false, {{"fused", 1}, {"separate", 0}, {nullptr, 0}}},
     {"pool", "PNVO_POOL", &PnvoOptions::pool, false, {{"fused", 1}, {"separate", 0}, {nullptr, 0}}},
@@ -1545,7 +1592,20 @@
 int run_fc_rows(pnvo_handle m, pnvo_handle const *grp, const int *end, int ng, int B, const float *comp_raw, const float *sc, const float *sh,
                 const FwdRequest &r);
 
+int forward_layers(pnvo_handle m, int B, const FwdRequest &r);
+
 int forward_body(pnvo_handle m, int B, const FwdRequest &r) {
+  m->chain_pending.clear();
+  m->chain_log.clear();
+  m->chain_on = m->opt.chain && !m->timing && m->tap_dst == nullptr && m->train == nullptr && r.grp == nullptr && m->precision == 0;
+  int rc = forward_layers(m, B, r);
+  if (rc == PNVO_OK) rc = pnvo_chain_flush(m, r.s);
+  m->chain_pending.clear();
+  m->chain_on = false;
+  return rc;
+}
+
+int forward_layers(pnvo_handle m, int B, const FwdRequest &r) {
   const pnvo_config &c = m->cfg;
   const GroupedFwd *grp = r.grp;
   hipStream_t s = r.s;
@@ -1610,6 +1670,7 @@
                                          .ss = m->ssA, .grp = grp, .s = s})) != PNVO_OK)
         return rc;
       const long Pb = (long)b3.hout * b3.wout;
+      if ((rc = pnvo_chain_flush(m, s)) != PNVO_OK) return rc;
       if (ds) {
         const Layer &cd = m->convs[b.ds];
         if ((rc = pnvo_run_conv(m, cd, B, {.x = cur, .y = m->rawD, .y_cstride = cd.coutp, .ss = m->ssD, .grp = grp, .s = s})) != PNVO_OK)
@@ -1650,6 +1711,7 @@
     if (c2_small_generic) {
       float *napp = ds_ride ? nxt : m->rawD;
       {
+        if ((rc = pnvo_chain_flush(m, s)) != PNVO_OK) return rc;
         Timed t(m, s, "gn_relu_apply", 0.0, 8.0 * B * P * c2.cinp);
         HIPCHK(m, launch_apply_ss_relu(m->rawA, m->ssA[0], m->ssA[1], B, P, c2.cinp, napp, s));
       }
@@ -1673,6 +1735,7 @@
       have_tail = true;
       continue;
     }
+    if ((rc = pnvo_chain_flush(m, s)) != PNVO_OK) return rc;
     {
       Timed t(m, s, "residual", 0.0, 12.0 * B * P * c2.coutp);
       HIPCHK(m, launch_residual(m->rawB, m->ssB[0], m->ssB[1], ds ? m->rawD : cur, ds ? m->ssD[0] : nullptr, ds ? m->ssD[1] : nullptr, B,
@@ -1692,6 +1755,7 @@
   } else if ((rc = pnvo_run_conv(m, comp, B, {.x = cur, .y = m->comp_raw, .y_cstride = comp.coutp, .ss = m->ssC, .grp = grp, .s = s})) != PNVO_OK) {
     return rc;
   }
+  if ((rc = pnvo_chain_flush(m, s)) != PNVO_OK) return rc;
   if (m->tap_dst != nullptr && m->tap_name == "compression") {
     HIPCHK(m, launch_apply_ss_relu(m->comp_raw, m->ssC[0], m->ssC[1], B, (long)m->fh * m->fw, m->comp_cp, m->tapbuf, s));
     if ((rc = maybe_tap(m, "compression", m->tapbuf, (size_t)B * m->fh * m->fw * m->comp_cp, s)) != PNVO_OK) return rc;
@@ -2269,6 +2333,12 @@
   return fail(h, PNVO_ERR_ARG, std::string("no residual-stage conv named '") + name + "'");
 }
 
+int pnvo_last_chains(pnvo_handle h, char *buf, size_t cap) {
+  if (!h) return 0;
+  if (buf != nullptr && cap > 0) std::snprintf(buf, cap, "%s", h->chain_log.c_str());
+  return (int)h->chain_log.size();
+}
+
 int pnvo_timing_mode(pnvo_handle h, int mode) {
   if (!h) return fail(h, PNVO_ERR_ARG, "null handle");
   h->timing = mode ? 1 : 0;
diff --git a/pointnav-vo_amd/csrc/pnvo_model.h b/pointnav-vo_amd/csrc/pnvo_model.h
--- a/pointnav-vo_amd/csrc/pnvo_model.h
+++ b/pointnav-vo_amd/csrc/pnvo_model.h
@@ -50,11 +50,13 @@
   int x3_strip = 1;
   int x3_fine = 1;
   int x3_w8 = 1;
+  int x3_w8s = 1;
   int x3_ksplit = 1;
   int fc_rows = 48;
   int head_fuse = 1;
   int ds_fuse = 1;
   int gn_fuse = 1;
+  int chain = 1;
   int x3_s2 = 1;
   int tail = 1;
   int pool = 1;
@@ -167,6 +169,16 @@
   int graph_mode = -1;
   unsigned long long graph_clock = 0;
 
+  struct ChainPending {
+    pnvo::ConvX3Args a;
+    int rows, kind, ks, stride, mode, mw, nw;
+    size_t ldsb;
+    const Layer *layer;
+  };
+  std::vector<ChainPending> chain_pending;
+  bool chain_on = false;
+  std::string chain_log;
+
   int timing = 0;
   std::vector<pnvo_kernel_time> tentries;
   std::map<std::string, int> tindex;
@@ -259,6 +271,7 @@
 };
 
 int pnvo_run_conv(pnvo_handle m, const Layer &l, int B, const ConvRequest &r);
+int pnvo_chain_flush(pnvo_handle m, hipStream_t s);
 bool pnvo_conv_takes_ds(pnvo_handle m, const Layer &c1, const Layer &cd, int B);
 bool pnvo_conv_on_x3(pnvo_handle m, const Layer &l, int B);
 bool pnvo_conv_takes_tail(pnvo_handle m, const Layer &l, int B);
diff --git a/pointnav-vo_amd/vo_cnn.py b/pointnav-vo_amd/vo_cnn.py
--- a/pointnav-vo_amd/vo_cnn.py
+++ b/pointnav-vo_amd/vo_cnn.py
@@ -289,6 +289,13 @@
         _lib.check(_lib.lib.pnvo_layer_kernel(self._handle, name.encode(), int(batch), buf, 32, C.byref(fl)), self._handle)
         return buf.value.decode(), float(fl.value)
 
+    def last_chains(self):
+        if self._handle is None:
+            return []
+        buf = C.create_string_buffer(2048)
+        _lib.lib.pnvo_last_chains(self._handle, buf, 2048)
+        return [c.split("+") for c in buf.value.decode().split(";") if c]
+
     def timing(self, enable):
         dev = next(self.parameters()).device
         self._ensure_handle(dev)
```
